# infergo-ml/gogp

Hardware: AMD Instinct MI355X
Metric: GP.Observe+Gradient evals/sec (fp64) at N=16384 D=8 (higher is better)
Workload: dtype f64

## Files before the change

### gogp_amd/_lib.py

```python
from __future__ import annotations

import ctypes
import os
import subprocess

from .kernel import CDesc

_HERE = os.path.dirname(os.path.abspath(__file__))
LIB_PATH = os.path.join(_HERE, "libgogp_hip.so")
HOOKS_PATH = os.path.join(_HERE, "libgogp_testhooks.so")

GOGP_OK, GOGP_EARG, GOGP_ENOTPD, GOGP_EHIP, GOGP_ESTATE, GOGP_ENOMEM, GOGP_ECOND = 0, 1, 2, 3, 4, 5, 6
GOGP_MAX_CANDIDATES = 16
GOGP_BATCH_MAX_N = 128
GOGP_COV_MAX_M = 4096

_dp = ctypes.POINTER(ctypes.c_double)
_i64 = ctypes.c_int64
_h = ctypes.c_void_p
_descp = ctypes.POINTER(CDesc)
GOGP_UNIQUE_ID_BYTES = 128


class CXfer(ctypes.Structure):
    _fields_ = [("peer", ctypes.c_int32), ("is_send", ctypes.c_int32), ("buf", ctypes.c_void_p),
                ("bytes", ctypes.c_int64)]


EXCHANGE_FN = ctypes.CFUNCTYPE(ctypes.c_int, ctypes.c_void_p, ctypes.POINTER(CXfer), ctypes.c_int32)
ALLREDUCE_FN = ctypes.CFUNCTYPE(ctypes.c_int, ctypes.c_void_p, ctypes.POINTER(ctypes.c_double),
                                ctypes.c_int64)
class CGemmOpts(ctypes.Structure):
    _fields_ = [(n, ctypes.c_int32) for n in ("ktri", "krag0", "new_row0", "kbeg0", "small_below", "prio", "rule",
                                              "tpb_shift", "rblk0", "cblk0", "pr", "Pr", "pc", "Pc", "beta0", "k")]
    _fields_ += [("bstride", ctypes.c_int64)]
    DEFAULTS = dict(ktri=0, krag0=-1, new_row0=-1, kbeg0=0, small_below=384, prio=0, rule=0, tpb_shift=0, rblk0=0,
                    cblk0=0, pr=0, Pr=1, pc=0, Pc=1, beta0=-1, k=1, bstride=0)


class CKParams(ctypes.Structure):
    _T, _D, _E = 4, 64, 32
    _fields_ = [("ndim", ctypes.c_int32), ("nterms", ctypes.c_int32), ("kind", ctypes.c_int32 * _T),
                ("ard", ctypes.c_int32 * _T), ("c", ctypes.c_double * _T), ("w", ctypes.c_double * _T),
                ("inv_len", (ctypes.c_double * _D) * _T), ("noise_var", ctypes.c_double), ("dnoise", ctypes.c_double),
                ("nevents", ctypes.c_int32), ("ev_axis", ctypes.c_int32), ("ev_from", ctypes.c_double * _E),
                ("ev_to", ctypes.c_double * _E), ("ev_disc", ctypes.c_double * _E)]


GOGP_TEST_NACC = 16 + 64


class CGemmPlan(ctypes.Structure):
    _fields_ = [("tile", ctypes.c_int32), ("waves", ctypes.c_int32), ("grid_x", ctypes.c_int64),
                ("grid_z", ctypes.c_int64), ("flops", ctypes.c_double), ("tag", ctypes.c_int64)]


SYMBOLS = [
    ("gogp_desc_check", ctypes.c_int, [_descp]),
    ("gogp_desc_ntheta_noise", ctypes.c_int, [_descp]),
    ("gogp_create", ctypes.c_int, [_descp, ctypes.c_int, ctypes.POINTER(_h)]),
    ("gogp_destroy", None, [_h]),
    ("gogp_last_error", ctypes.c_char_p, [_h]),
    ("gogp_notpd_index", _i64, [_h]),
    ("gogp_graph_info", ctypes.c_int, [_h, ctypes.POINTER(ctypes.c_int64), ctypes.POINTER(ctypes.c_int)]),
    ("gogp_events_check", ctypes.c_int, [_dp, ctypes.c_int, ctypes.c_int, ctypes.c_int]),
    ("gogp_set_events", ctypes.c_int, [_h, _dp, ctypes.c_int, ctypes.c_int]),
    ("gogp_set_data", ctypes.c_int, [_h, _dp, _dp, _i64]),
    ("gogp_set_data_device", ctypes.c_int, [_h, ctypes.c_void_p, ctypes.c_void_p, _i64]),
    ("gogp_absorb", ctypes.c_int, [_h, _dp, _dp]),
    ("gogp_observe", ctypes.c_int, [_h, _dp, _i64, _dp]),
    ("gogp_observe_full", ctypes.c_int, [_h, _dp, _i64, _dp]),
    ("gogp_lml", ctypes.c_int, [_h, _dp]),
    ("gogp_gradient", ctypes.c_int, [_h, _dp, _i64]),
    ("gogp_loo", ctypes.c_int, [_h, _dp, _dp, _dp, _dp]),
    ("gogp_loo_gradient", ctypes.c_int, [_h, _dp, _i64]),
    ("gogp_observe_gradient_batch", ctypes.c_int,
     [ctypes.POINTER(_h), ctypes.c_int, _dp, _i64, _dp, _dp, ctypes.POINTER(ctypes.c_int)]),
    ("gogp_observe_gradient_candidates", ctypes.c_int,
     [_h, ctypes.c_int, _dp, _i64, _dp, _dp, ctypes.POINTER(ctypes.c_int)]),
    ("gogp_batch_set_data", ctypes.c_int,
     [_h, _dp, _dp, _i64, ctypes.c_int32, ctypes.POINTER(_i64), ctypes.POINTER(_i64)]),
    ("gogp_batch_observe_gradient", ctypes.c_int,
     [_h, ctypes.c_int32, ctypes.POINTER(ctypes.c_int32), _dp, _i64, _dp, _dp, ctypes.POINTER(ctypes.c_int)]),
    ("gogp_batch_produce", ctypes.c_int,
     [_h, ctypes.c_int32, ctypes.POINTER(ctypes.c_int32), _dp, _i64, ctypes.POINTER(_i64), _dp, _dp, _dp, _dp,
      ctypes.POINTER(ctypes.c_int)]),
    ("gogp_batch_observe_full_gradient", ctypes.c_int,
     [_h, ctypes.c_int32, _dp, ctypes.POINTER(_i64), _dp, _dp, ctypes.POINTER(ctypes.c_int)]),
    ("gogp_batch_produce_full", ctypes.c_int,
     [_h, ctypes.c_int32, _dp, ctypes.POINTER(_i64), ctypes.POINTER(_i64), _dp, _dp, _dp, _dp,
      ctypes.POINTER(ctypes.c_int)]),
    ("gogp_produce", ctypes.c_int, [_h, _dp, _i64, _dp, _dp]),
    ("gogp_produce_gradient", ctypes.c_int, [_h, _dp, _i64, _dp, _dp, _dp, _dp]),
    ("gogp_produce_covariance", ctypes.c_int, [_h, _dp, _i64, _dp, _dp]),
    ("gogp_produce_samples", ctypes.c_int, [_h, _dp, _i64, _dp, _i64, ctypes.c_double, _dp, _dp]),
    ("gogp_n", _i64, [_h]),
    ("gogp_get_alpha", ctypes.c_int, [_h, _dp]),
    ("gogp_get_factor", ctypes.c_int, [_h, _dp]),
    ("gogp_get_factor_rows", ctypes.c_int, [_h, ctypes.POINTER(_i64), _i64, _dp]),
    ("gogp_get_factor_diag", ctypes.c_int, [_h, _dp]),
    ("gogp_set_factor", ctypes.c_int, [_h, _dp, _dp, _dp, _dp]),
    ("gogp_append", ctypes.c_int, [_h, _dp, _dp, ctypes.c_int64]),
    ("gogp_remove", ctypes.c_int, [_h, ctypes.POINTER(_i64), ctypes.c_int64]),
    ("gogp_dist_grid", ctypes.c_int, [ctypes.c_int, ctypes.POINTER(ctypes.c_int), ctypes.POINTER(ctypes.c_int)]),
    ("gogp_dist_unique_id", ctypes.c_int, [ctypes.c_void_p]),
    ("gogp_dist_init_rccl", ctypes.c_int,
     [_h, ctypes.c_int, ctypes.c_int, ctypes.c_int, ctypes.c_int, ctypes.c_char_p]),
    ("gogp_dist_init_callbacks", ctypes.c_int,
     [_h, ctypes.c_int, ctypes.c_int, ctypes.c_int, ctypes.c_int, ctypes.c_void_p, ctypes.c_void_p,
      ctypes.c_void_p]),
    ("gogp_dist_local_bytes", _i64, [_h]),
    ("gogp_dist_comm_ranks", ctypes.c_int, [_h, ctypes.POINTER(ctypes.c_int)]),
    ("gogp_dist_selftest", ctypes.c_int, [_h, ctypes.c_int, _i64]),
    ("gogp_profile_enable", ctypes.c_int, [_h, ctypes.c_int]),
    ("gogp_profile_read", ctypes.c_int, [_h, _dp, ctypes.POINTER(_i64), _dp, _dp]),
    ("gogp_profile_read_launches", ctypes.c_int,
     [_h, _i64, _dp, _dp, _dp, ctypes.POINTER(_i64), ctypes.POINTER(_i64)]),
    ("gogp_profile_read_aux", ctypes.c_int, [_h, ctypes.c_int, _dp, ctypes.POINTER(_i64)]),
    ("gogp_set_option", ctypes.c_int, [_h, ctypes.c_char_p, _i64]),
    ("gogp_version", ctypes.c_char_p, []),
# ... 107 lines not shown
```

### gogp_amd/csrc/api.hip

```cpp
#include <math.h>
#include <stdio.h>
#include <stdlib.h>
#include <string.h>

#include <algorithm>
#include <initializer_list>
#include <mutex>
#include <new>
#include <thread>
#include <type_traits>
#include <utility>

#include "handle.h"

using namespace gogp;

static thread_local std::string g_create_error;

extern "C" int gogp_desc_ntheta_noise(const gogp_desc *d) {
  return (d && (d->noise_kind == GOGP_NOISE_UNIFORM || d->noise_kind == GOGP_NOISE_CONSTANT_PARAM)) ? 1 : 0;
}

extern "C" int gogp_desc_check(const gogp_desc *d) {
  if (!d) return GOGP_EARG;
  if (d->ndim < 1 || d->ndim > GOGP_MAX_NDIM) return GOGP_EARG;
  if (d->nterms < 1 || d->nterms > GOGP_MAX_TERMS) return GOGP_EARG;
  if (d->ntheta_simil < 1 || d->ntheta_simil > GOGP_MAX_NDIM + 8) return GOGP_EARG;
  if (d->noise_kind != GOGP_NOISE_CONSTANT && d->noise_kind != GOGP_NOISE_UNIFORM &&
      d->noise_kind != GOGP_NOISE_CONSTANT_PARAM)
    return GOGP_EARG;
  int nard = 0;
  for (int t = 0; t < d->nterms; ++t) {
    const gogp_term &T = d->terms[t];
    if (T.kind < GOGP_K_NORMAL || T.kind > GOGP_K_PERIODIC) return GOGP_EARG;
    if (T.scale_idx >= d->ntheta_simil || T.scale_idx < -1) return GOGP_EARG;
    const int nlen = T.ard ? d->ndim : 1;
    if (T.len_idx < 0 || T.len_idx + nlen > d->ntheta_simil) return GOGP_EARG;
    if (T.kind == GOGP_K_PERIODIC) {
      if (T.period_idx < 0 || T.period_idx >= d->ntheta_simil) return GOGP_EARG;
      if (!(T.period_mult > 0)) return GOGP_EARG;
    }
    if (T.ard) ++nard;
  }
  if (nard > 1) return GOGP_EARG;
  return GOGP_OK;
}

extern "C" int gogp_events_check(const double *events, int nevents, int axis, int ndim) {
  if (nevents < 0 || nevents > GOGP_MAX_EVENTS) return GOGP_EARG;
  if (ndim < 1 || ndim > GOGP_MAX_NDIM || axis < 0 || axis >= ndim) return GOGP_EARG;
  if (nevents > 0 && !events) return GOGP_EARG;
  for (int i = 0; i < 3 * nevents; ++i)
    if (!isfinite(events[i])) return GOGP_EARG;
  return GOGP_OK;
}

extern "C" const char *gogp_version(void) {
#ifndef GOGP_BUILD_ID
#define GOGP_BUILD_ID "unknown"
#endif
  return "gogp_hip 0.3 gfx950 fp64-mfma(v_mfma_f64_16x16x4_f64) tile128 panel256 build " GOGP_BUILD_ID;
}

extern "C" const char *gogp_last_error(const gogp_handle *h) {
  if (!h) return g_create_error.c_str();
  return h->err.c_str();
}

extern "C" int64_t gogp_notpd_index(const gogp_handle *h) { return h ? h->notpd : -1; }
extern "C" int64_t gogp_n(const gogp_handle *h) { return h ? h->n : 0; }

static void free_n_buffers(gogp_handle *h) {
  nbufs_free(nbufs_of(h));
  nbufs_put(h, NBufs());
  (void)hipFree(h->bufY);
  h->bufY = nullptr;
  (void)hipFree(h->rw);
  (void)hipFree(h->rz);
  (void)hipFree(h->rd);
  (void)hipFree(h->rpart);
  h->small_ws.release();
  h->app_ws.release();
  h->rm_ws.release();
  h->loo_vec.release();
  h->loo_mat.release();
  (void)hipFree(h->TX);
  (void)hipFree(h->Tmt);
  h->TX = h->Tmt = nullptr;
  h->cap_tinv = 0;
  h->tinv_valid = h->tinv_pending = false;
  (void)hipFree(h->g32A);
  (void)hipFree(h->g32L);
  (void)hipFree(h->g32Y);
  (void)hipFree(h->g32D);
  h->g32A = h->g32L = h->g32Y = h->g32D = nullptr;
  h->g32_cap = 0;
  h->rw = h->rz = h->rd = h->rpart = nullptr;
  h->cap_npad = 0;
  h->cap_y = 0;
}

static void drop_cand_graph(gogp_handle *h) {
  if (h->cand_graph) (void)hipGraphExecDestroy(h->cand_graph);
  h->cand_graph = nullptr;
  h->cand_seen_key = CandGraphKey();
}
static hipError_t graph_stream(gogp_handle *h);

static void free_cand_buffers(gogp_handle *h) {
  drop_cand_graph(h);
  (void)hipFree(h->cand_arena);
  (void)hipHostFree(h->cand_hostP);
  (void)hipHostFree(h->cand_hscal);
  h->cand_arena = nullptr;
  h->cand_hostP = nullptr;
  h->cand_hscal = nullptr;
  h->cand_stride = 0;
  h->cand_cap_k = h->cand_host_k = 0;
  h->cand_cap_npad = 0;
}

static void free_m_buffers(gogp_handle *h) {
  (void)hipFree(h->dZ);
  (void)hipFree(h->KsT);
  (void)hipFree(h->Vt);
  (void)hipFree(h->pvec);
  h->pg_ws.release();
  h->pc_ws.release();
  h->dZ = h->KsT = h->Vt = h->pvec = nullptr;
  h->cap_m = h->cap_mp_npad = 0;
}

struct StreamSet {
  int device = -1;
  bool in_use = false;
  hipStream_t s = nullptr, s2 = nullptr, sp = nullptr, st = nullptr, sl = nullptr, sk = nullptr;
  hipStream_t sg = nullptr;
};
static std::mutex g_pool_mutex;
static std::vector<StreamSet *> g_stream_pool;

static hipError_t create_stream_set(StreamSet *ss, int device) {
  ss->device = device;
  hipError_t e = hipSuccess;
  e = hipStreamCreateWithFlags(&ss->s, hipStreamNonBlocking);
  if (e == hipSuccess) e = hipStreamCreateWithFlags(&ss->s2, hipStreamNonBlocking);
  if (e == hipSuccess) {
    int least = 0, greatest = 0;
    (void)hipDeviceGetStreamPriorityRange(&least, &greatest);
    const int normal = (least + greatest) / 2;
    e = hipStreamCreateWithPriority(&ss->sp, hipStreamNonBlocking, greatest);
    if (e == hipSuccess) e = hipStreamCreateWithPriority(&ss->st, hipStreamNonBlocking, normal);
    if (e == hipSuccess) e = hipStreamCreateWithPriority(&ss->sl, hipStreamNonBlocking, normal);
    if (e == hipSuccess) e = hipStreamCreateWithPriority(&ss->sk, hipStreamNonBlocking, least);
  }
  return e;
}

static hipError_t acquire_streams(gogp_handle *h, int device) {
  std::lock_guard<std::mutex> lock(g_pool_mutex);
  StreamSet *ss = nullptr;
  for (StreamSet *c : g_stream_pool)
    if (!c->in_use && c->device == device) {
      ss = c;
      break;
    }
  if (!ss) {
    ss = new StreamSet();
    const hipError_t e = create_stream_set(ss, device);
    if (e != hipSuccess) {
      for (hipStream_t q : {ss->s, ss->s2, ss->sp, ss->st, ss->sl, ss->sk})
        if (q) (void)hipStreamDestroy(q);
      delete ss;
      return e;
    }
    g_stream_pool.push_back(ss);
  }
  ss->in_use = true;
  h->stream_set = ss;
  h->s = ss->s;
  h->s2 = ss->s2;
  h->sp = ss->sp;
  h->st = ss->st;
  h->sl = ss->sl;
  h->sk = ss->sk;
  return hipSuccess;
}

static hipError_t graph_stream(gogp_handle *h) {
  StreamSet *ss = static_cast<StreamSet *>(h->stream_set);
  if (!ss->sg) {
    const hipError_t e = hipStreamCreateWithFlags(&ss->sg, hipStreamNonBlocking);
    if (e != hipSuccess) return e;
  }
  h->sg = ss->sg;
  return hipSuccess;
}

static void release_streams(gogp_handle *h) {
  std::lock_guard<std::mutex> lock(g_pool_mutex);
  if (h->stream_set) static_cast<StreamSet *>(h->stream_set)->in_use = false;
  h->stream_set = nullptr;
// ... 161 lines not shown
    for (int f = 0; f < 3; ++f) h->events[e][f] = events[3 * e + f];
  h->factored = h->have_alpha = h->have_kinv = h->observed = h->grad_valid = false;
  h->trtri_done = h->trtri_pending = h->alpha_pending = h->kinv_pending = false;
  h->tinv_valid = h->tinv_pending = false;
  return GOGP_OK;
}

static void fill_params_theta(const gogp_handle *h, const double *ts, const double *tn, DevParams &p) {
  const gogp_desc &d = h->desc;
  memset(&p, 0, sizeof p);
  p.ndim = d.ndim;
  p.nterms = d.nterms;
  p.ns = h->ns;
  p.nn = h->nn;
  for (int t = 0; t < d.nterms; ++t) {
    const gogp_term &T = d.terms[t];
    p.kind[t] = T.kind;
    p.ard[t] = T.ard;
    p.c[t] = T.scale_idx >= 0 ? ts[T.scale_idx] : 1.0;
    p.w[t] = 0.0;
    if (T.kind == GOGP_K_PERIODIC)
      p.w[t] = M_PI / (T.period_mult * ts[T.period_idx]);
    for (int j = 0; j < d.ndim; ++j)
      p.inv_len[t][j] = 1.0 / ts[T.len_idx + (T.ard ? j : 0)];
  }
  if (d.noise_kind == GOGP_NOISE_CONSTANT || d.noise_kind == GOGP_NOISE_CONSTANT_PARAM) {
    p.noise_var = d.noise_std * d.noise_std;
    p.dnoise = 0.0;
  } else {
    const double sd = tn[0];
    p.noise_var = d.noise_scale * sd * sd;
    p.dnoise = 2.0 * p.noise_var;
  }
  p.nevents = h->nevents;
  p.ev_axis = h->ev_axis;
  for (int e = 0; e < h->nevents; ++e) {
    p.ev_from[e] = h->events[e][0];
    p.ev_to[e] = h->events[e][1];
    p.ev_disc[e] = h->events[e][2];
  }
}

static void fill_params(const gogp_handle *h, DevParams &p) {
  fill_params_theta(h, h->theta_s.data(), h->theta_n.data(), p);
}

int gogp_upload_params(gogp_handle *h) {
  if (h->batch_mode) return GOGP_OK;
  fill_params(h, *h->hostP);
  HIPCHK(h, hipMemcpyAsync(h->devP, h->hostP, sizeof(DevParams), hipMemcpyHostToDevice, h->s));
  return GOGP_OK;
}

static hipError_t cand_memset(gogp_handle *h, void *dst, size_t bytes, hipStream_t s) {
  hipError_t e = hipSuccess;
  for (int c = 0; c < h->batch_k && e == hipSuccess; ++c)
    e = gogp::rec_memset_async((char *)dst + (size_t)c * h->cand_stride, 0, bytes, s);
  return e;
}
static hipError_t cand_copy_in(gogp_handle *h, void *dst, const void *src, size_t bytes, hipStream_t s) {
  hipError_t e = hipSuccess;
  for (int c = 0; c < h->batch_k && e == hipSuccess; ++c)
    e = gogp::rec_memcpy_async((char *)dst + (size_t)c * h->cand_stride, src, bytes, hipMemcpyDeviceToDevice, s);
  return e;
}
static hipError_t cand_d2h(gogp_handle *h, double *hdst, const void *dsrc, size_t bytes, hipStream_t s) {
  hipError_t e = hipSuccess;
  for (int c = 0; c < h->batch_k && e == hipSuccess; ++c)
    e = gogp::rec_memcpy_async(hdst + (size_t)c * BATCH_ROW, (const char *)dsrc + (size_t)c * h->cand_stride, bytes,
                               hipMemcpyDeviceToHost, s);
  return e;
}

static int ensure_y(gogp_handle *h) {
  if (h->bufY && h->cap_y >= h->npad) return GOGP_OK;
  (void)hipFree(h->bufY);
  h->bufY = nullptr;
  h->cap_y = 0;
  const int64_t cap = std::max(h->npad, h->cap_npad);
  HIPCHK(h, hipMalloc(&h->bufY, (size_t)cap * (size_t)cap * h->esz()));
  h->cap_y = cap;
  return GOGP_OK;
}

static int ensure_d64(gogp_handle *h) {
  if (h->D64 && h->cap_d64 >= h->npad) return GOGP_OK;
  (void)hipFree(h->D64);
  h->D64 = nullptr;
  h->cap_d64 = 0;
  const int64_t cap = std::max(h->npad, h->cap_npad);
  HIPCHK(h, hipMalloc(&h->D64, (size_t)cap * PANEL * sizeof(double)));
  h->cap_d64 = cap;
  return GOGP_OK;
}

struct FactorResult {
  int rc = GOGP_OK;
  double lml = 0.0, cond_lb = 1.0, yta = 0.0;
  int64_t notpd = -1;
  std::string msg;
};
static FactorResult judge_scalars(const gogp_handle *h, const double *hs, bool fp32, bool refine, int64_t n = -1) {
  FactorResult r;
  long long info = 0;
  memcpy(&info, hs + HS_INFO, sizeof info);
  char buf[160];
  if (info != 0) {
    r.rc = GOGP_ENOTPD;
    r.notpd = (int64_t)info - 1;
    snprintf(buf, sizeof buf, "Factorize: matrix is not positive definite (pivot %lld)", (long long)r.notpd);
    r.msg = buf;
    return r;
  }
  const double logdet = fp32 ? hs[5] : hs[0];
  const double ztz = refine ? hs[6] : hs[1];
  r.yta = ztz;
  r.lml = -0.5 * (double)(n < 0 ? h->n : n) * log(2 * M_PI) - 0.5 * logdet - 0.5 * ztz;
  const double dmin = hs[3], dmax = hs[4];
  r.cond_lb = (dmin > 0.0) ? (dmax / dmin) * (dmax / dmin) : INFINITY;
  if (!(r.cond_lb <= h->cond_limit)) {
    snprintf(buf, sizeof buf, "Condition: matrix singular or near-singular with condition number >= %.4e",
             r.cond_lb);
    r.msg = buf;
    r.rc = GOGP_ECOND;
  }
  return r;
}

static int finish_factorize(gogp_handle *h, bool fp32, bool refine, bool kinv) {
  h->alpha_pending = true;
  if (h->batch_mode) {
    h->factored = h->have_alpha = true;
    if (kinv) h->have_kinv = true;
    return GOGP_OK;
  }
  HIPCHK(h, hipStreamSynchronize(h->s));
  HIPCHK(h, hipGetLastError());
  const FactorResult fr = judge_scalars(h, h->hscal, fp32, refine);
  if (fr.rc == GOGP_ENOTPD) {
    h->alpha_pending = h->kinv_pending = false;
    h->tinv_valid = h->tinv_pending = false;
    h->trtri_done = h->trtri_pending = false;
    h->notpd = fr.notpd;
    h->err = fr.msg;
    return GOGP_ENOTPD;
  }
  h->lml = fr.lml;
  h->yta = fr.yta;
  h->factored = h->have_alpha = true;
  h->z_valid = true;
  if (kinv) h->have_kinv = true;
  h->cond_lb = fr.cond_lb;
  if (fr.rc == GOGP_ECOND) h->err = fr.msg;
  return fr.rc;
}

static void diag_block(gogp_handle *h, hipStream_t sp, const double *A, int64_t ld, double *L, int64_t ldl,
                       double *Dp, int64_t c0) {
  launch_diag256(sp, A, ld, L, ldl, Dp, c0, h->n, h->info);
}
static void diag_block(gogp_handle *h, hipStream_t sp, const float *A, int64_t ld, float *L, int64_t ldl,
                       float *Dp, int64_t c0) {
  double *A64 = h->dscr, *L64 = h->dscr + PANEL * PANEL, *D64 = h->dscr + 2 * PANEL * PANEL;
  if (h->d64_active)
    A64 = h->D64 + (size_t)(c0 / PANEL) * PANEL * PANEL;
  else
    launch_convert_block(sp, A, ld, A64, PANEL, PANEL, PANEL);
  launch_diag256(sp, A64, PANEL, L64, PANEL, D64, c0, h->n, h->info);
  launch_convert_block(sp, L64, PANEL, L, ldl, PANEL, PANEL);
  launch_convert_block(sp, D64, PANEL, Dp, PANEL, PANEL, PANEL);
  launch_logdet_block(sp, L64, PANEL, c0, h->n, PANEL, h->scalars + 5);
}
static void diag_inv_only(gogp_handle *h, hipStream_t s, const double *L, int64_t ld, double *Dp) {
  (void)h;
  launch_diag256_inv_only(s, L, ld, Dp);
}
static void diag_inv_only(gogp_handle *h, hipStream_t s, const float *L, int64_t ld, float *Dp) {
  double *L64 = h->dscr + PANEL * PANEL, *D64 = h->dscr + 2 * PANEL * PANEL;
  launch_convert_block(s, L, ld, L64, PANEL, PANEL, PANEL);
  launch_diag256_inv_only(s, L64, PANEL, D64);
  launch_convert_block(s, D64, PANEL, Dp, PANEL, PANEL, PANEL);
}

static inline int chain_prio_of(const gogp_handle *h) {
  return h->chain_prio < 0 ? (h->npad <= 6144 ? 1 : 0) : h->chain_prio;
}
static inline GemmGrid chain_grid(const gogp_handle *h) {
  GemmGrid g;
  g.prio = chain_prio_of(h);
  return g;
}

static inline int superpanel_width(const gogp_handle *h, int npanel, int P0) {
  const int head = h->superpanel_head < 0 ? (h->prec == 32 ? 4 : 3) : h->superpanel_head;
  const int sw = (head > 0 && npanel - P0 > h->head_remaining) ? head : h->superpanel;
  return (npanel - P0 < sw) ? npanel - P0 : sw;
}
struct SuperPanel {
  int P0, nsub, prevP0, next_nsub;
  int64_t C0() const { return (int64_t)P0 * PANEL; }
  int64_t CE() const { return C0() + (int64_t)nsub * PANEL; }
};
static std::vector<SuperPanel> superpanels(const gogp_handle *h) {
  const int npanel = (int)(h->npad / PANEL);
  std::vector<SuperPanel> v;
  for (int P0 = 0; P0 < npanel; P0 += v.back().nsub) {
    const int nsub = superpanel_width(h, npanel, P0);
    if (!v.empty()) v.back().next_nsub = nsub;
    v.push_back({P0, nsub, v.empty() ? -1 : v.back().P0, 0});
  }
  return v;
}
struct InnerGroup {
  int grp;
  int64_t k0, ce;
};
static inline InnerGroup inner_group(int q, int64_t c2, int64_t CE) {
  const int done = q + 1, grp = done & -done;
  return {grp, c2 - (int64_t)grp * PANEL, std::min(c2 + (int64_t)grp * PANEL, CE)};
}

constexpr int TMT_BLOCKS = 8;
static inline int tinv_panels(const gogp_handle *h) { return h->produce_panels; }
static inline int64_t tinv_signature(const gogp_handle *h) {
  return (int64_t)h->produce_panels + (h->npad << 8) + ((int64_t)h->prec << 56);
}
static int ensure_tinv(gogp_handle *h) {
  const int64_t tld = (int64_t)tinv_panels(h) * PANEL;
  const size_t need = (size_t)std::max(h->npad, h->cap_npad) * (size_t)tld;
  if (!h->TX || h->cap_tinv < need) {
    (void)hipFree(h->TX);
    (void)hipFree(h->Tmt);
    h->TX = h->Tmt = nullptr;
    h->cap_tinv = 0;
    HIPCHK(h, hipMalloc(&h->TX, need * h->esz()));
    HIPCHK(h, hipMalloc(&h->Tmt, (size_t)TMT_BLOCKS * PANEL * PANEL * h->esz()));
    h->cap_tinv = need;
  }
  h->tinv_ld = tld;
  return GOGP_OK;
}

template <class T>
static void assemble_tinv(gogp_handle *h, hipStream_t sp, int P0, int nsub) {
  const int64_t ld = h->npad, tld = h->tinv_ld, C0 = (int64_t)P0 * PANEL;
  T *X = reinterpret_cast<T *>(h->TX) + C0 * tld;
  T *MT = reinterpret_cast<T *>(h->Tmt);
  const T *L = reinterpret_cast<const T *>(h->bufL);
  const T *Dinv = reinterpret_cast<const T *>(h->Dinv) + (size_t)P0 * PANEL * PANEL;
  launch_tinv_init(sp, Dinv, X, (T *)nullptr, nsub, tld);
  for (int d = 1; d < nsub; ++d) {
    const int cnt = nsub - d;
    for (int b0 = 0; b0 < cnt; b0 += 6) {
      const int nb = std::min(6, cnt - b0);
      const T *A1[6], *B1[6], *A2[6], *B2[6];
      T *C1[6], *C2[6];
      int64_t lda1[6], ldb1[6], ldc1[6], lda2[6], ldb2[6], ldc2[6];
      int K1[6], K2[6];
      for (int b = 0; b < nb; ++b) {
        const int i = d + b0 + b, j = i - d;
        A1[b] = L + (C0 + (int64_t)i * PANEL) * ld + C0 + (int64_t)j * PANEL;
        lda1[b] = ld;
        B1[b] = X + (int64_t)j * PANEL * tld + (int64_t)j * PANEL;
        ldb1[b] = tld;
        C1[b] = MT + (size_t)(b0 + b) * PANEL * PANEL;
        ldc1[b] = PANEL;
        K1[b] = d * PANEL;
        A2[b] = Dinv + (size_t)i * PANEL * PANEL;
        lda2[b] = PANEL;
        B2[b] = C1[b];
        ldb2[b] = PANEL;
        C2[b] = X + (int64_t)i * PANEL * tld + (int64_t)j * PANEL;
        ldc2[b] = tld;
        K2[b] = PANEL;
      }
      launch_blockmm(sp, nb, A1, lda1, B1, ldb1, C1, ldc1, K1, 1.0);
      launch_blockmm(sp, nb, A2, lda2, B2, ldb2, C2, ldc2, K2, -1.0);
    }
  }
}

template <class T>
struct InvBufs {
  T *A, *Y;
  const T *L, *Dinv;
};
template <class T>
static void trtri_superstep(gogp_handle *h, const InvBufs<T> &B, const SuperPanel &P, hipStream_t st, hipStream_t s2) {
  const int64_t npad = h->npad, ld = npad;
  T *R = B.A, *Y = B.Y;
  const T *L = B.L;
  GemmProfile *pf = &h->prof;
  const int P0 = P.P0;
  const int64_t C0 = P.C0(), CE = P.CE();
  for (int q = 0; q < P.nsub; ++q) {
    const int p = P0 + q;
    const int64_t c0 = (int64_t)p * PANEL, c2 = c0 + PANEL;
    const T *Dp = B.Dinv + (size_t)p * PANEL * PANEL;
    launch_ydiag(st, Dp, Y + c0 * ld + c0, ld);
    if (c2 < CE)
      launch_zero_block(st, Y + c2 * ld + c0, ld, CE - c2, PANEL);
    if (c0 > 0) {
      GemmGrid gtri = chain_grid(h);
      gtri.ktri = h->ktri;
      launch_gemm_nt(st, GEMM_RECT, (int)(c0 / TILE), 2, PANEL, 1.0, R + c0, ld, Dp, PANEL, 0.0,
                      Y + c0, ld, pf, &gtri);
    }
    if (c2 < CE) {
      const InnerGroup g = inner_group(q, c2, CE);
      GemmGrid gch = chain_grid(h);
      if (h->krag) gch.krag0 = (int)(g.k0 / TILE);
      launch_gemm_nt(st, GEMM_RECT, (int)(c2 / TILE), (int)((g.ce - c2) / TILE), (int64_t)g.grp * PANEL,
                      -1.0, Y + g.k0, ld, L + c2 * ld + g.k0, ld, 1.0, R + c2, ld, pf, &gch);
    }
  }
  order(h, EV_BASE + 4 * P0 + 2, st, s2);
  const int nt = (int)((npad - CE) / TILE);
  if (nt > 0) {
    const int64_t Kw = CE - C0;
    const int mr = (int)(CE / TILE);
    const int ntn = nt < 2 * P.next_nsub ? nt : 2 * P.next_nsub;
    if (P0 > 0 && st != s2)
      (void)gogp::rec_stream_wait(st, ev(h, EV_BASE + 4 * P.prevP0 + 3));
    GemmGrid gch = chain_grid(h), gbulk;
    if (h->krag) gch.krag0 = gbulk.krag0 = (int)(C0 / TILE);
    launch_gemm_nt(st, GEMM_RECT, mr, ntn, Kw, -1.0, Y + C0, ld, L + CE * ld + C0, ld, 1.0,
                    R + CE, ld, pf, &gch);
    if (nt > ntn) {
      const int64_t C3 = CE + (int64_t)ntn * TILE;
      launch_gemm_nt(s2, GEMM_RECT, mr, nt - ntn, Kw, -1.0, Y + C0, ld, L + C3 * ld + C0, ld, 1.0,
                      R + C3, ld, pf, &gbulk);
    }
    (void)gogp::rec_event_record(ev(h, EV_BASE + 4 * P0 + 3), s2);
  }
}

static inline bool mixed_gradient(const gogp_handle *h) {
  return h->grad_prec == 32 && h->prec == 64 && !h->batch_mode && !h->dist;
}
static int ensure_g32(gogp_handle *h) {
  const int64_t cap = std::max(h->npad, h->cap_npad);
  if (h->g32A && h->g32_cap >= cap) return GOGP_OK;
  (void)hipFree(h->g32A);
  (void)hipFree(h->g32L);
  (void)hipFree(h->g32Y);
  (void)hipFree(h->g32D);
  h->g32A = h->g32L = h->g32Y = h->g32D = nullptr;
  h->g32_cap = 0;
  const size_t nn = (size_t)cap * (size_t)cap * sizeof(float);
  HIPCHK(h, hipMalloc(&h->g32A, nn));
  HIPCHK(h, hipMalloc(&h->g32L, nn));
  HIPCHK(h, hipMalloc(&h->g32Y, nn));
  HIPCHK(h, hipMalloc(&h->g32D, (size_t)(cap / PANEL) * PANEL * PANEL * sizeof(float)));
  h->g32_cap = cap;
  return GOGP_OK;
}
static void mixed_superstep(gogp_handle *h, const SuperPanel &P, hipStream_t st, hipStream_t s2) {
  const int64_t npad = h->npad, ld = npad, C0 = P.C0(), W = P.CE() - C0;
  launch_convert_block(st, h->bufL + C0 * ld + C0, ld, h->g32L + C0 * ld + C0, ld, (int)(npad - C0), (int)W);
  launch_convert_block(st, h->Dinv + (size_t)P.P0 * PANEL * PANEL, PANEL, h->g32D + (size_t)P.P0 * PANEL * PANEL, PANEL,
                       (int)W, PANEL);
  const InvBufs<float> B{h->g32A, h->g32Y, h->g32L, h->g32D};
  trtri_superstep<float>(h, B, P, st, s2);
}

template <class T>
static void kinv_accumulate(gogp_handle *h, const T *Y, T *A, int64_t C0, int64_t CE) {
  (void)gogp::rec_stream_wait(h->sk, ev(h, EV_BASE + 4 * (size_t)(C0 / PANEL) + 2));
  GemmGrid gk;
  gk.new_row0 = (int)(C0 / TILE);
  if (h->krag) gk.krag0 = (int)(C0 / TILE);
  launch_gemm_nt(h->sk, GEMM_LOWER, (int)(CE / TILE), (int)(CE / TILE), CE - C0, 1.0, Y + C0, h->npad, Y + C0, h->npad,
                 1.0, A, h->npad, &h->prof, &gk);
}

template <class T>
static void zero_inverse_rhs(gogp_handle *h, bool mixed, hipStream_t s) {
  if (mixed)
    launch_zero_upper_blocks(s, h->g32A, h->npad, h->npad);
  else
    launch_zero_upper_blocks(s, reinterpret_cast<T *>(h->bufA), h->npad, h->npad);
}
template <class T>
static void inverse_superstep(gogp_handle *h, bool mixed, const SuperPanel &P, hipStream_t st, hipStream_t s2,
                              bool fuse_kinv) {
  if (mixed) {
    mixed_superstep(h, P, st, s2);
    if (fuse_kinv) kinv_accumulate<float>(h, h->g32Y, h->g32A, P.C0(), P.CE());
  } else {
    const InvBufs<T> B{reinterpret_cast<T *>(h->bufA), reinterpret_cast<T *>(h->bufY), reinterpret_cast<const T *>(h->bufL),
                       reinterpret_cast<const T *>(h->Dinv)};
    trtri_superstep<T>(h, B, P, st, s2);
    if (fuse_kinv) kinv_accumulate<T>(h, B.Y, B.A, P.C0(), P.CE());
  }
}

static inline int chain_split_of(const gogp_handle *h, bool eager) {
  if (h->dist || h->prec != 64) return 0;
  if (h->chain_split >= 0) return h->chain_split;
  return (h->npad <= 8192 || !eager) ? 2 : 0;
}
static void fused_panel(gogp_handle *h, hipStream_t sp, double *A, double *L, int64_t ld, int64_t c0, int64_t npad,
                        GemmProfile *pf) {
  const int64_t c1 = c0 + TILE, c2 = c0 + PANEL;
  const int mt1 = (int)((npad - c1) / TILE);
  const GemmGrid gch = chain_grid(h);
  launch_panel128_slabs(sp, A + c0 * ld + c0, ld, L + c0 * ld + c0, ld, 0, npad - c1, c0, h->n, h->info, h->chain_slabs);
  launch_gemm_nt(sp, GEMM_RECT, mt1, 1, TILE, -1.0, L + c1 * ld + c0, ld, L + c1 * ld + c0, ld, 1.0, A + c1 * ld + c1, ld,
                 pf, &gch);
  launch_panel128_slabs(sp, A + c0 * ld + c0, ld, L + c0 * ld + c0, ld, 1, npad - c2, c0, h->n, h->info, h->chain_slabs);
}

static void begin_evaluation(gogp_handle *h, std::initializer_list<hipStream_t> streams) {
  auto wait = [&](int e) {
    for (hipStream_t q : streams) (void)gogp::rec_stream_wait(q, ev(h, e));
  };
  if (h->trtri_pending) wait(EV_TRTRI);
  if (h->kinv_pending) wait(EV_KINV);
  if (h->kinv_c1 > 0 && !h->have_kinv) wait(EV_KINV);
  h->trtri_pending = h->kinv_pending = false;
  h->factored = h->have_alpha = h->have_kinv = h->grad_valid = false;
  h->alpha_pending = h->trtri_done = h->ydone_valid = h->d64_active = false;
  h->notpd = -1;
  h->kinv_c1 = 0;
  if (!h->batch_mode) h->tinv_valid = false;
}
static hipError_t enqueue_result_scalars(gogp_handle *h, hipStream_t s) {
  const hipError_t e = cand_d2h(h, h->hscal, h->scalars, 7 * sizeof(double), s);
  return e != hipSuccess ? e : cand_d2h(h, h->hscal + HS_INFO, h->info, sizeof(long long), s);
}

template <class T>
static void substitute_fwd(gogp_handle *h, hipStream_t q, const T *L, const T *Dinv, double *w, double *dst) {
  const int npanel = (int)(h->npad / PANEL);
  for (int b = 0; b < npanel; ++b) launch_trsv_fwd_step(q, L, h->npad, Dinv, b, npanel, w, dst);
}
template <class T>
static hipError_t substitute_bwd(gogp_handle *h, hipStream_t q, const T *L, const T *Dinv, const double *src, double *w,
                                 double *dst) {
  const int npanel = (int)(h->npad / PANEL);
  const hipError_t e = hipMemcpyAsync(w, src, (size_t)h->npad * sizeof(double), hipMemcpyDeviceToDevice, q);
  for (int b = npanel - 1; b >= 0 && e == hipSuccess; --b) launch_trsv_bwd_step(q, L, h->npad, Dinv, b, npanel, w, dst);
  return e;
}

template <class T>
struct Sweep {
  static constexpr bool fp32 = sizeof(T) == 4;
  gogp_handle *h;
  bool eager;
  T *A = reinterpret_cast<T *>(h->bufA), *L = reinterpret_cast<T *>(h->bufL), *Dinv = reinterpret_cast<T *>(h->Dinv);
  int64_t npad = h->npad, ld = npad;
  int npanel = (int)(npad / PANEL);
  GemmProfile *pf = &h->prof;
  hipStream_t s = h->s, st = h->st, s2 = h->s2;
  hipStream_t sp = h->lookahead ? h->sp : h->s;
  hipStream_t sz = h->lookahead ? h->sl : sp;
  bool mixed = !fp32 && mixed_gradient(h);
  bool fuse_kinv = eager && (h->kinv_fused < 0 ? (npad <= 10240 || mixed) : h->kinv_fused != 0);
  int split = fp32 ? 0 : chain_split_of(h, eager);

  void d64_init(hipStream_t q, int first, int nblk) const {
    if constexpr (fp32)
      launch_widen_diag_blocks(q, A + (int64_t)first * PANEL * (ld + 1), ld, h->D64 + (size_t)first * PANEL * PANEL, nblk);
  }
  void d64_update(hipStream_t q, int64_t k0, int64_t K, int first, int nblk) const {
    if constexpr (fp32) {
      if (h->d64_active)
        launch_diag_syrk_f64(q, L + (int64_t)first * PANEL * ld + k0, ld, K, h->D64 + (size_t)first * PANEL * PANEL, nblk);
    }
  }

  int build_gram() const {
    if (sp != s) order(h, EV_ENTRY, s, sp);
    HIPCHK(h, cand_memset(h, h->info, sizeof(long long), sp));
    const int w0 = superpanel_width(h, npanel, 0);
    {
      AuxTimer tm(h, GOGP_PROF_GRAM, s);
      launch_gram_lower_split(sp, s, h->devP, h->D, h->dX, h->n, npad, A, ld, (int64_t)w0 * PANEL, h->ev());
    }
    h->d64_active = fp32 && h->diag_fp64 != 0;
    if (h->d64_active) {
      const int rc = ensure_d64(h);
      if (rc != GOGP_OK) return rc;
      d64_init(sp, 0, w0);
      if (npanel > w0) d64_init(s, w0, npanel - w0);
    }
    (void)gogp::rec_event_record(ev(h, EV_GRAM), s);
    if (eager) {
      (void)gogp::rec_stream_wait(s2, ev(h, EV_GRAM));
      (void)gogp::rec_stream_wait(st, ev(h, EV_GRAM));
      zero_inverse_rhs<T>(h, mixed, s2);
      order(h, EV_INIT, s2, st);
    }
    return GOGP_OK;
  }

  void chain_superpanel(const SuperPanel &P) const {
    const int64_t CE = P.CE();
    for (int q = 0; q < P.nsub; ++q) {
      const int p = P.P0 + q;
      const int64_t c0 = (int64_t)p * PANEL, c2 = c0 + PANEL;
      if constexpr (!fp32) {
        if (split) fused_panel(h, sp, A, L, ld, c0, npad, pf);
      }
      if (!split) {
        T *Dp = Dinv + (size_t)p * PANEL * PANEL;
        diag_block(h, sp, A + c0 * ld + c0, ld, L + c0 * ld + c0, ld, Dp, c0);
        const int mt2 = (int)((npad - c2) / TILE);
        if (mt2 > 0) {
          GemmGrid gtri = chain_grid(h);
          gtri.ktri = h->ktri;
          launch_gemm_nt(sp, GEMM_RECT, mt2, 2, PANEL, 1.0, A + c2 * ld + c0, ld, Dp, PANEL, 0.0,
                          L + c2 * ld + c0, ld, pf, &gtri);
        }
      }
      if (c2 < CE) {
        d64_update(sp, c0, PANEL, p + 1, (int)((CE - c2) / PANEL));
        const InnerGroup g = inner_group(q, c2, CE);
        const GemmGrid gch = chain_grid(h);
        launch_gemm_nt(sp, GEMM_TRAP, (int)((npad - c2) / TILE), (int)((g.ce - c2) / TILE),
                        (int64_t)g.grp * PANEL, -1.0, L + c2 * ld + g.k0, ld, L + c2 * ld + g.k0, ld, 1.0,
                        A + c2 * ld + c2, ld, pf, &gch);
      }
    }
  }

  void panels_final(const SuperPanel &P) const {
    order(h, EV_BASE + 4 * P.P0, sp, s);
    if (sz != sp) (void)gogp::rec_stream_wait(sz, ev(h, EV_BASE + 4 * P.P0));
    if constexpr (!fp32) {
      if (split) {
        launch_dinv256_blocks(sz, L + (int64_t)P.P0 * PANEL * (ld + 1), ld, Dinv + (size_t)P.P0 * PANEL * PANEL, P.nsub);
        if (eager) {
          (void)gogp::rec_event_record(ev(h, EV_BASE + 5 * (size_t)npanel + 32 + (size_t)P.P0), sz);
          (void)gogp::rec_stream_wait(st, ev(h, EV_BASE + 5 * (size_t)npanel + 32 + (size_t)P.P0));
        }
      }
    }
    for (int q = 0; q < P.nsub; ++q) launch_trsv_fwd_step(sz, L, ld, Dinv, P.P0 + q, npanel, h->w, h->z);
  }

  void trailing_update(const SuperPanel &P) const {
    const int64_t C0 = P.C0(), CE = P.CE();
    const int mtE = (int)((npad - CE) / TILE);
    if (mtE <= 0) return;
    const int64_t Kw = CE - C0;
    const int ntn = mtE < 2 * P.next_nsub ? mtE : 2 * P.next_nsub;
    (void)gogp::rec_stream_wait(sp, ev(h, P.P0 > 0 ? EV_BASE + 4 * P.prevP0 + 1 : EV_GRAM));
    const GemmGrid gch = chain_grid(h);
    launch_gemm_nt(sp, GEMM_TRAP, mtE, ntn, Kw, -1.0, L + CE * ld + C0, ld, L + CE * ld + C0, ld,
                    1.0, A + CE * ld + CE, ld, pf, &gch);
    d64_update(sp, C0, Kw, (int)(CE / PANEL), ntn / 2);
    if (mtE > ntn) {
      const int64_t C3 = CE + (int64_t)ntn * TILE;
      launch_gemm_nt(s, GEMM_LOWER, mtE - ntn, mtE - ntn, Kw, -1.0, L + C3 * ld + C0, ld,
                      L + C3 * ld + C0, ld, 1.0, A + C3 * ld + C3, ld, pf);
      d64_update(s, C0, Kw, (int)(C3 / PANEL), (mtE - ntn) / 2);
    }
    (void)gogp::rec_event_record(ev(h, EV_BASE + 4 * P.P0 + 1), s);
  }

  void inverse_behind(const SuperPanel &P) const {
    const int64_t CE = P.CE();
    (void)gogp::rec_stream_wait(st, ev(h, EV_BASE + 4 * P.P0));
    inverse_superstep<T>(h, mixed, P, st, s2, fuse_kinv);
    if (!fp32 && !fuse_kinv && !mixed && !h->batch_mode && h->kinv_split > 0 && h->kinv_c1 == 0 && CE < npad &&
        CE * 100 >= npad * (int64_t)h->kinv_split) {
      (void)gogp::rec_stream_wait(h->sk, ev(h, EV_BASE + 4 * P.P0 + 2));
      const T *Y0 = reinterpret_cast<const T *>(h->bufY);
      launch_gemm_nt(h->sk, GEMM_LAUUM, (int)(CE / TILE), (int)(CE / TILE), CE, 1.0, Y0, ld, Y0, ld, 0.0, A, ld, pf);
      (void)gogp::rec_event_record(ev(h, EV_KINV), h->sk);
      h->kinv_c1 = CE;
    }
  }

  int finish_alpha() const {
    if (fp32) {
      if (sz != sp) (void)gogp::rec_stream_wait(sp, ev(h, EV_FWD));
      HIPCHK(h, substitute_bwd(h, sp, L, Dinv, h->z, h->w, h->alpha));
      for (int it = 0; it < h->refine_steps; ++it) {
        launch_residual(sp, h->devP, h->D, h->dX, h->n, npad, h->alpha, h->dy, h->rpart, REFINE_SLABS, h->rw,
                        h->radial1, h->ev());
        substitute_fwd(h, sp, L, Dinv, h->rw, h->rz);
        HIPCHK(h, substitute_bwd(h, sp, L, Dinv, h->rz, h->rw, h->rd));
        launch_axpy(sp, h->alpha, h->rd, npad);
      }
      launch_dot(sp, h->dy, h->alpha, h->n, h->scalars + 6);
      order(h, EV_ALPHA, sp, s);
    }
    HIPCHK(h, enqueue_result_scalars(h, s));
    if (fp32) {
      if (eager) (void)gogp::rec_event_record(ev(h, EV_TRTRI), st);
    } else if (eager && !mixed) {
      (void)gogp::rec_stream_wait(st, ev(h, EV_FWD));
      launch_alpha_from_y(st, reinterpret_cast<const T *>(h->bufY), ld, h->z, npad, h->alpha);
      (void)gogp::rec_event_record(ev(h, EV_ALPHA), st);
      (void)gogp::rec_event_record(ev(h, EV_TRTRI), st);
    } else {
      if (sz != sp) (void)gogp::rec_stream_wait(sp, ev(h, EV_FWD));
      HIPCHK(h, substitute_bwd(h, sp, L, Dinv, h->z, h->w, h->alpha));
      (void)gogp::rec_event_record(ev(h, EV_ALPHA), sp);
    }
    return GOGP_OK;
  }
};

template <class T>
static int factorize_t(gogp_handle *h, bool eager) {
  const Sweep<T> c{h, eager && h->lookahead != 0};
  begin_evaluation(h, {c.s, c.sp});
  int rc = gogp_upload_params(h);
  if (rc == GOGP_OK && (c.mixed || c.eager)) rc = c.mixed ? ensure_g32(h) : ensure_y(h);
  if (rc == GOGP_OK) rc = c.build_gram();
  if (rc != GOGP_OK) return rc;
  if (c.fp32) HIPCHK(h, hipMemsetAsync(h->scalars + 5, 0, sizeof(double), c.sp));
  HIPCHK(h, cand_copy_in(h, h->w, h->dy, (size_t)c.npad * sizeof(double), c.sp));
  if (c.sz != c.sp) order(h, EV_W, c.sp, c.sz);
  for (const SuperPanel &P : superpanels(h)) {
    c.chain_superpanel(P);
    c.panels_final(P);
    c.trailing_update(P);
    if (c.eager) c.inverse_behind(P);
  }
  if (c.fuse_kinv) {
    (void)gogp::rec_event_record(ev(h, EV_KINV), h->sk);
    h->kinv_pending = true;
  }
  if (c.eager) {
    (void)gogp::rec_event_record(ev(h, EV_TRTRI), c.st);
    (void)gogp::rec_event_record(ev(h, EV_YDONE), c.st);
    h->ydone_valid = h->trtri_done = h->trtri_pending = true;
  }
  order(h, EV_FWD, c.sz, c.s);
  launch_lml_scalars(c.s, c.L, c.ld, h->z, nullptr, nullptr, h->n, h->scalars);
  rc = c.finish_alpha();
  if (rc != GOGP_OK) return rc;
  const int rcf = finish_factorize(h, c.fp32, c.fp32, false);
  if (rcf == GOGP_ENOTPD)
    for (hipStream_t q : {c.sp, c.st, c.s2, h->sl, h->sk}) (void)hipStreamSynchronize(q);
  return rcf;
}

static inline bool tiny_ok(const gogp_handle *h) {
  return h->tiny && !h->dist && h->prec == 64 && h->npad == PANEL && h->n <= TILE && !mixed_gradient(h);
}
static int tiny_factorize(gogp_handle *h, bool eager) {
  hipStream_t s = h->s;
  begin_evaluation(h, {s});
  int rc = gogp_upload_params(h);
  if (rc != GOGP_OK) return rc;
  if (h->lookahead && !h->batch_mode) {
    order(h, EV_ENTRY, h->sp, s);
    order(h, EV_W, h->sl, s);
  }
  HIPCHK(h, cand_memset(h, h->info, sizeof(long long), s));
  launch_tiny_eval(s, h->devP, h->dX, h->dy, h->n, h->bufA, h->bufL, h->Dinv, h->z, h->alpha, h->info, eager, h->ev());
  launch_lml_scalars(s, h->bufL, h->npad, h->z, nullptr, nullptr, h->n, h->scalars);
  (void)gogp::rec_event_record(ev(h, EV_ALPHA), s);
  HIPCHK(h, enqueue_result_scalars(h, s));
  return finish_factorize(h, false, false, eager);
}

static int factorize(gogp_handle *h, bool eager) {
  if (tiny_ok(h)) return tiny_factorize(h, eager && h->lookahead);
  return h->prec == 32 ? factorize_t<float>(h, eager) : factorize_t<double>(h, eager);
}

static int ensure_alpha(gogp_handle *h) {
  if (!h->factored || !h->have_alpha) return fail(h, GOGP_ESTATE, "no factorisation");
  if (h->alpha_pending) {
    HIPCHK(h, gogp::rec_stream_wait(h->s, ev(h, EV_ALPHA)));
    h->alpha_pending = false;
  }
  return GOGP_OK;
}

static const char *theta_refusal(const gogp_handle *h, const double *ts, const double *tn) {
  for (int i = 0; i < h->ns; ++i)
    if (!(ts[i] > 0.0) || !std::isfinite(ts[i])) return "similarity parameters must be positive and finite";
  for (int i = 0; i < h->nn; ++i)
    if (!std::isfinite(tn[i])) return "noise parameter must be finite";
  return nullptr;
}

static int set_theta_natural(gogp_handle *h, const double *ts, const double *tn) {
  if (const char *why = theta_refusal(h, ts, tn)) return fail(h, GOGP_EARG, why);
  for (int i = 0; i < h->ns; ++i) h->theta_s[i] = ts[i];
  for (int i = 0; i < h->nn; ++i) h->theta_n[i] = tn[i];
  h->have_theta = true;
  return GOGP_OK;
}

extern "C" int gogp_absorb(gogp_handle *h, const double *theta_simil,
                           const double *theta_noise) {
  if (!h || !theta_simil || (h->nn > 0 && !theta_noise)) return fail(h, GOGP_EARG, "absorb: NULL");
// ... 12 lines not shown
  rc = h->dist ? gogp_dist_factorize(h, false) : factorize(h, false);
  if (rc != GOGP_OK && rc != GOGP_ECOND) return rc;
  const int rcond = rc;
  rc = ensure_alpha(h);
  if (rc != GOGP_OK) return rc;
  HIPCHK(h, hipStreamSynchronize(h->s));
  return rcond;
}

static int observe_theta(gogp_handle *h, const double *x, double *lml) {
  std::vector<double> th(h->P > 0 ? h->P : 1);
  for (int i = 0; i < h->P; ++i) th[i] = exp(x[i]);
  int rc = set_theta_natural(h, th.data(), th.data() + h->ns);
  if (rc != GOGP_OK) return rc;
  h->grad_valid = false;
  if (h->n == 0) {
    h->lml = 0.0;
    h->factored = false;
    h->observed = true;
    if (lml) *lml = 0.0;
    return GOGP_OK;
  }
  rc = h->dist ? gogp_dist_factorize(h, true)
               : factorize(h, h->eager != 0);
  if (rc != GOGP_OK && rc != GOGP_ECOND) return rc;
  h->observed = true;
  if (lml) *lml = h->lml;
  return rc;
}

extern "C" int gogp_observe(gogp_handle *h, const double *x, int64_t len, double *lml) {
  if (!h || !x) return fail(h, GOGP_EARG, "observe: NULL");
  if (len != h->P) return fail(h, GOGP_EARG, "len(x)");
  if (!h->have_data) return fail(h, GOGP_ESTATE, "observe: no data (gogp_set_data)");
  HIPCHK(h, hipSetDevice(h->device));
  h->with_obs = false;
  return observe_theta(h, x, lml);
}

extern "C" int gogp_observe_full(gogp_handle *h, const double *x, int64_t len, double *lml) {
  if (!h || !x) return fail(h, GOGP_EARG, "observe: NULL");
  if (len < h->P) return fail(h, GOGP_EARG, "len(x)");
  const int64_t rest = len - h->P;
  if (rest == 0) return gogp_observe(h, x, len, lml);
  const int64_t n = rest / (h->D + 1);
  if (n * (h->D + 1) != rest) return fail(h, GOGP_EARG, "len(x)");
  int rc = gogp_set_data(h, x + h->P, x + h->P + n * h->D, n);
  if (rc != GOGP_OK) return rc;
  h->with_obs = true;
  return observe_theta(h, x, lml);
}

extern "C" int gogp_lml(gogp_handle *h, double *lml) {
  if (!h || !lml) return GOGP_EARG;
  if (h->n == 0) {
    *lml = 0.0;
    return GOGP_OK;
  }
  if (!h->factored) return fail(h, GOGP_ESTATE, "LML: nothing absorbed");
  *lml = h->lml;
  return GOGP_OK;
}

template <class T>
static int compute_kinv_t(gogp_handle *h) {
  if (h->have_kinv) return GOGP_OK;
  const int64_t npad = h->npad, ld = npad;
  hipStream_t s = h->s;
  GemmProfile *pf = &h->prof;
  if (h->kinv_pending) {
    (void)gogp::rec_stream_wait(s, ev(h, EV_KINV));
    if (h->trtri_pending) (void)gogp::rec_stream_wait(s, ev(h, EV_TRTRI));
    h->kinv_pending = h->trtri_pending = false;
    h->have_kinv = true;
    return GOGP_OK;
  }
  const bool mixed = std::is_same<T, double>::value && mixed_gradient(h);
  if (!h->trtri_done) {
    hipStream_t sp = h->lookahead ? h->sp : h->s;
    const int rcy = mixed ? ensure_g32(h) : ensure_y(h);
    if (rcy != GOGP_OK) return rcy;
    zero_inverse_rhs<T>(h, mixed, s);
    order(h, EV_INIT, s, sp);
    for (const SuperPanel &P : superpanels(h)) inverse_superstep<T>(h, mixed, P, sp, s, false);
    order(h, EV_TRTRI, sp, s);
    h->trtri_done = true;
  } else if (h->trtri_pending) {
    (void)gogp::rec_stream_wait(s, ev(h, h->ydone_valid ? EV_YDONE : EV_TRTRI));
  }
  if (mixed) {
    launch_gemm_nt(s, GEMM_LAUUM, h->nblk, h->nblk, npad, 1.0, h->g32Y, ld, h->g32Y, ld, 0.0, h->g32A, ld, pf);
  } else {
    GemmGrid gk;
    if (h->kinv_c1 > 0) {
      (void)gogp::rec_stream_wait(s, ev(h, EV_KINV));
      gk.kbeg0 = (int)h->kinv_c1;
    }
    launch_gemm_nt(s, GEMM_LAUUM, h->nblk, h->nblk, npad, 1.0, reinterpret_cast<const T *>(h->bufY), ld,
                   reinterpret_cast<const T *>(h->bufY), ld, 0.0, reinterpret_cast<T *>(h->bufA), ld, pf, &gk);
  }
  if (h->trtri_pending && h->ydone_valid) (void)gogp::rec_stream_wait(s, ev(h, EV_TRTRI));
  h->trtri_pending = false;
  h->have_kinv = true;
  return GOGP_OK;
}
static int compute_kinv(gogp_handle *h) {
  return h->prec == 32 ? compute_kinv_t<float>(h) : compute_kinv_t<double>(h);
}

static int64_t grad_len(const gogp_handle *h) {
  return h->with_obs ? h->P + h->n * (h->D + 1) : h->P;
}

static void assemble_gradient(const gogp_handle *h, const double *a, double dnoise, double *out) {
  const gogp_desc &d = h->desc;
  for (int t = 0; t < d.nterms; ++t) {
    const gogp_term &T = d.terms[t];
    if (T.scale_idx >= 0) out[T.scale_idx] += 0.5 * a[3 * t + 0];
    if (T.ard) {
      for (int j = 0; j < d.ndim; ++j) out[T.len_idx + j] += 0.5 * a[ACC_ARD0 + j];
    } else {
      out[T.len_idx] += 0.5 * a[3 * t + 1];
    }
    if (T.kind == GOGP_K_PERIODIC) out[T.period_idx] += 0.5 * a[3 * t + 2];
  }
  if (h->nn > 0) out[h->ns] = 0.5 * a[ACC_TRACE] * dnoise;
}

static void fp32_gradient_identities(const gogp_handle *h, double *a, double trace_w, double yta, double noise_var) {
  const gogp_desc &d = h->desc;
  a[ACC_TRACE] = trace_w;
  if (d.nterms == 1 && d.terms[0].scale_idx >= 0) a[0] = (yta - (double)h->n) - noise_var * trace_w;
}

static int enqueue_grad_sums(gogp_handle *h, bool trace) {
  hipStream_t s = h->s;
  auto reduce = [&](auto *kinv) {
    AuxTimer tm(h, GOGP_PROF_GRAD, s);
    launch_grad_reduce(s, h->devP, h->D, h->ard_dims, h->dX, h->alpha, kinv, h->npad, h->n, h->npad, h->gpart, h->gout,
                       h->radial1, h->ard_mfma_min, h->ev());
  };
  if (h->prec == 32)
    reduce(reinterpret_cast<const float *>(h->bufA));
  else if (mixed_gradient(h))
    reduce((const float *)h->g32A);
  else
    reduce((const double *)h->bufA);
  HIPCHK(h, cand_d2h(h, h->hscal + HS_GRAD, h->gout, NACC * sizeof(double), s));
  h->hscal[HS_TRACE] = NAN;
  if (trace) {
    launch_trace_from_y(s, h->prec == 32 ? reinterpret_cast<const float *>(h->bufY) : (const float *)h->g32Y, h->npad, h->n,
                        h->npad, h->alpha, h->prec == 32 ? h->rw : h->w, h->scalars + 7);
    HIPCHK(h, hipMemcpyAsync(h->hscal + HS_TRACE, h->scalars + 7, sizeof(double), hipMemcpyDeviceToHost, s));
  }
  return GOGP_OK;
}

extern "C" int gogp_gradient(gogp_handle *h, double *grad, int64_t len) {
  if (!h || !grad) return fail(h, GOGP_EARG, "gradient: NULL");
  if (!h->observed) return fail(h, GOGP_ESTATE, "Gradient before Observe");
  if (len != grad_len(h)) return fail(h, GOGP_EARG, "gradient: wrong length");
  for (int64_t i = 0; i < len; ++i) grad[i] = 0.0;
  if (h->n == 0) return GOGP_OK;
  HIPCHK(h, hipSetDevice(h->device));
  if (h->dist && h->with_obs)
    return fail(h, GOGP_EARG, "sharded evaluation: the full Observe form is not supported");
  if (h->prec == 32 && h->with_obs)
// ... 107 lines not shown
  if (rc != GOGP_OK) return rc;
  for (int64_t i = 0; i < len; ++i) grad[i] = 0.0;
  if (empty) return GOGP_OK;
  hipStream_t s = h->s;
  const int64_t npad = h->npad, ld = npad;
  const size_t mat = (size_t)npad * (size_t)npad;
  rc = h->loo_mat.reserve(h, 2 * mat * sizeof(double));
  if (rc != GOGP_OK) return rc;
  double *B = h->loo_mat.as<double>(), *G = B + mat;
  launch_loo_scale_symv(s, h->bufA, ld, h->n, npad, lv.sc, lv.v, B, ld, G, lv.u);
  launch_gemm_nt(s, GEMM_LOWER, h->nblk, h->nblk, npad, 1.0, (const double *)B, ld, (const double *)B, ld, 0.0, G, ld,
                 &h->prof);
  launch_loo_rank2(s, G, ld, h->n, npad, lv.u, h->alpha);
  HIPCHK(h, hipMemsetAsync(lv.zero, 0, (size_t)npad * sizeof(double), s));
  {
    AuxTimer tm(h, GOGP_PROF_GRAD, s);
    launch_grad_reduce(s, h->devP, h->D, h->ard_dims, h->dX, lv.zero, (const double *)G, ld, h->n, npad, h->gpart, h->gout,
                       h->radial1, h->ard_mfma_min, h->ev());
  }
  double acc[NACC];
  HIPCHK(h, hipMemcpyAsync(acc, h->gout, sizeof acc, hipMemcpyDeviceToHost, s));
  HIPCHK(h, hipStreamSynchronize(s));
  HIPCHK(h, hipGetLastError());
  assemble_gradient(h, acc, h->hostP->dnoise, grad);
  return GOGP_OK;
}

static int fill_params_log(const gogp_handle *h, const double *x, DevParams &p) {
  std::vector<double> th((size_t)std::max(h->P, 1));
  for (int i = 0; i < h->P; ++i) th[(size_t)i] = exp(x[i]);
  int rc = GOGP_OK;
  if (theta_refusal(h, th.data(), th.data() + h->ns)) {
    rc = GOGP_EARG;
    std::fill(th.begin(), th.end(), 1.0);
  }
  fill_params_theta(h, th.data(), th.data() + h->ns, p);
  return rc;
}

static int judge_row(const gogp_handle *h, double *row, bool fp32, int64_t n, const DevParams &p, int st,
                     const char *refused, double *lml, double *g, int64_t len, std::string &first_msg) {
  *lml = NAN;
  if (g) std::fill(g, g + len, 0.0);
  if (st != GOGP_OK) {
    if (first_msg.empty()) first_msg = refused;
    return st;
  }
  const FactorResult fr = judge_scalars(h, row, fp32, fp32, n);
  if (fr.rc != GOGP_OK && first_msg.empty()) first_msg = fr.msg;
  if (fr.rc != GOGP_ENOTPD) {
    *lml = fr.lml;
    if (fp32 && std::isfinite(row[HS_TRACE]))
      fp32_gradient_identities(h, row + HS_GRAD, row[HS_TRACE], fr.yta, p.noise_var);
    if (g) assemble_gradient(h, row + HS_GRAD, p.dnoise, g);
  }
  return fr.rc;
}

extern "C" int gogp_observe_gradient_batch(gogp_handle **hs, int k, const double *xs, int64_t len,
                                           double *lmls, double *grads, int *status) {
  if (!hs || k <= 0 || !xs || !lmls || !grads) return GOGP_EARG;
  std::vector<int> st((size_t)k, GOGP_OK);
  auto body = [&](int i) {
    int rc = gogp_observe(hs[i], xs + (size_t)i * len, len, lmls + i);
    if (rc == GOGP_OK) rc = gogp_gradient(hs[i], grads + (size_t)i * len, len);
    st[(size_t)i] = rc;
  };
  std::vector<std::thread> th;
  for (int i = 1; i < k; ++i) th.emplace_back(body, i);
  body(0);
  for (auto &t : th) t.join();
  int first = GOGP_OK;
  for (int i = 0; i < k; ++i) {
    if (status) status[i] = st[(size_t)i];
    if (first == GOGP_OK && st[(size_t)i] != GOGP_OK) first = st[(size_t)i];
  }
  return first;
}

static size_t align_up(size_t v, size_t a) { return (v + a - 1) / a * a; }
constexpr int64_t GRAPH_MAX_NPAD = 1024;
constexpr int64_t GRAPH_EXPLICIT_MAX_NPAD = 8192;

static EvalBufs cand_layout(char *base, int64_t npad, size_t esz, size_t *bytes = nullptr) {
  EvalBufs b;
  size_t o = 0;
  auto take = [&](auto *&p, size_t n) {
    p = reinterpret_cast<std::remove_reference_t<decltype(p)>>(reinterpret_cast<uintptr_t>(base) + o);
    o += align_up(n, 256);
  };
  const size_t nn = (size_t)npad * (size_t)npad * esz;
  take(b.devP, sizeof(DevParams));
  take(b.info, sizeof(long long));
  take(b.scalars, 8 * sizeof(double));
  take(b.gout, NACC * sizeof(double));
  take(b.z, (size_t)npad * sizeof(double));
  take(b.w, (size_t)npad * sizeof(double));
  take(b.alpha, (size_t)npad * sizeof(double));
  take(b.gpart, (size_t)grad_reduce_blocks(npad) * NACC * sizeof(double));
  take(b.Dinv, (size_t)(npad / PANEL) * PANEL * PANEL * esz);
  take(b.bufA, nn);
  take(b.bufL, nn);
  take(b.bufY, nn);
  if (bytes) *bytes = align_up(o, 4096);
  return b;
}

static int ensure_candidates(gogp_handle *h, int k) {
  if (k > h->cand_host_k) {
    drop_cand_graph(h);
    (void)hipHostFree(h->cand_hostP);
    (void)hipHostFree(h->cand_hscal);
    h->cand_hostP = nullptr;
    h->cand_hscal = nullptr;
    h->cand_host_k = 0;
    HIPCHK(h, hipHostMalloc((void **)&h->cand_hostP, (size_t)k * sizeof(DevParams), hipHostMallocDefault));
    HIPCHK(h, hipHostMalloc((void **)&h->cand_hscal, (size_t)k * BATCH_ROW * sizeof(double), hipHostMallocDefault));
    h->cand_host_k = k;
  }
  if (k > h->cand_cap_k || h->npad > h->cand_cap_npad) {
    drop_cand_graph(h);
    (void)hipFree(h->cand_arena);
    h->cand_arena = nullptr;
    h->cand_cap_k = 0;
    h->cand_cap_npad = 0;
    const int64_t cap = std::max(h->npad, h->cand_cap_npad);
    size_t stride = 0;
    (void)cand_layout(nullptr, cap, h->esz(), &stride);
    HIPCHK(h, hipMalloc((void **)&h->cand_arena, stride * (size_t)k));
    h->cand_stride = stride;
    h->cand_cap_k = k;
    h->cand_cap_npad = cap;
  }
  return GOGP_OK;
}

static CandGraphKey cand_graph_key(const gogp_handle *h, int k) {
  return {k, h->n, h->cand_cap_npad, h->cand_stride, h->cand_arena, h->dX, h->dy, h->cand_hostP, h->cand_hscal};
}

extern "C" int gogp_observe_gradient_candidates(gogp_handle *h, int k, const double *xs, int64_t len,
                                                double *lmls, double *grads, int *status) {
  if (!h || k <= 0 || !xs || !lmls || !grads) return fail(h, GOGP_EARG, "candidates: bad arguments");
  if (k > GOGP_MAX_CANDIDATES) return fail(h, GOGP_EARG, "candidates: k > GOGP_MAX_CANDIDATES");
  if (len != h->P) return fail(h, GOGP_EARG, "len(x)");
  if (!h->have_data) return fail(h, GOGP_ESTATE, "candidates: no data (gogp_set_data)");
  if (h->dist) {
    HIPCHK(h, hipSetDevice(h->device));
    for (int c = 0; c < k; ++c) {
      lmls[c] = NAN;
      if (status) status[c] = GOGP_ESTATE;
      for (int64_t i = 0; i < len; ++i) grads[(size_t)c * len + i] = 0.0;
    }
    int first_d = GOGP_OK;
    for (int c = 0; c < k; ++c) {
      double *g = grads + (size_t)c * len;
      h->with_obs = false;
      int r = observe_theta(h, xs + (size_t)c * len, &lmls[c]);
      if (r == GOGP_OK || r == GOGP_ECOND) {
        const int rg = gogp_gradient(h, g, len);
        if (rg != GOGP_OK) r = rg;
      }
      if (r == GOGP_ENOTPD || r == GOGP_EARG) {
        lmls[c] = NAN;
        for (int64_t i = 0; i < len; ++i) g[i] = 0.0;
      } else if (r != GOGP_OK && r != GOGP_ECOND) {
        return r;
      }
      if (status) status[c] = r;
      if (first_d == GOGP_OK && r != GOGP_OK) first_d = r;
    }
    return first_d;
  }
  if (h->prec == 32 && k > 1) {
    int first32 = GOGP_OK;
    for (int c = 0; c < k; ++c) {
      const int r = gogp_observe_gradient_candidates(h, 1, xs + (size_t)c * len, len, lmls + c, grads + (size_t)c * len,
                                                     status ? status + c : nullptr);
      if (r != GOGP_OK && r != GOGP_ENOTPD && r != GOGP_ECOND && r != GOGP_EARG) return r;
      if (first32 == GOGP_OK && r != GOGP_OK) first32 = r;
    }
    return first32;
  }
  if (!h->lookahead || !h->eager)
    return fail(h, GOGP_EARG, "candidates: needs the fused sweep (options lookahead and eager on)");
  if (h->n == 0) {
    for (int c = 0; c < k; ++c) {
      lmls[c] = 0.0;
      if (status) status[c] = GOGP_OK;
      for (int64_t i = 0; i < len; ++i) grads[(size_t)c * len + i] = 0.0;
    }
    return GOGP_OK;
  }
  HIPCHK(h, hipSetDevice(h->device));
  for (hipStream_t q : work_streams(h)) HIPCHK(h, hipStreamSynchronize(q));
  if (h->kinv_pending) h->have_kinv = true;
  h->trtri_pending = h->alpha_pending = h->kinv_pending = h->tinv_pending = false;
  int rc = ensure_candidates(h, k);
  if (rc != GOGP_OK) return rc;

  const EvalBufs saved_bufs = *h;
  const EvalState saved_state = *h;
  double *const saved_hscal = h->hscal;
  const int64_t saved_cap_y = h->cap_y;
  static_cast<EvalBufs &>(*h) = cand_layout(h->cand_arena, h->cand_cap_npad, h->esz());
  h->hscal = h->cand_hscal;
  h->cap_y = h->cand_cap_npad;
  h->with_obs = false;
  h->batch_k = k;
  h->batch_mode = true;
  gogp::tl_batch.k = k;
  gogp::tl_batch.stride = (long)h->cand_stride;
  std::vector<int> st((size_t)k, GOGP_OK);

  for (int c = 0; c < k; ++c) st[(size_t)c] = fill_params_log(h, xs + (size_t)c * len, h->cand_hostP[c]);
  auto enqueue = [&]() -> int {
    for (int c = 0; c < k; ++c)
      HIPCHK(h, gogp::rec_memcpy_async((char *)h->devP + (size_t)c * h->cand_stride, h->cand_hostP + c,
                                       sizeof(DevParams), hipMemcpyHostToDevice, h->s));
    const bool f32 = h->prec == 32;
    int r = tiny_ok(h) ? tiny_factorize(h, true) : (f32 ? factorize_t<float>(h, true) : factorize_t<double>(h, true));
    if (r != GOGP_OK) return r;
    r = f32 ? compute_kinv_t<float>(h) : compute_kinv_t<double>(h);
    if (r != GOGP_OK) return r;
    r = ensure_alpha(h);
    if (r != GOGP_OK) return r;
    r = enqueue_grad_sums(h, f32 && h->trace_fp64);
    if (r != GOGP_OK) return r;
    size_t slot = EV_BASE + 4 * (size_t)(h->npad / PANEL);
    for (hipStream_t q : {h->sp, h->s2, h->st, h->sl, h->sk}) order(h, slot++, q, h->s);
    return GOGP_OK;
  };
  auto run = [&]() -> int {
    int r = GOGP_OK;
    const bool dag = h->use_graph >= 2;
    const bool graph = h->use_graph && h->prec == 64 && !h->prof.on && !h->graph_failed &&
                       h->npad <= (dag ? GRAPH_EXPLICIT_MAX_NPAD : GRAPH_MAX_NPAD);
    const CandGraphKey key = cand_graph_key(h, k);
    const bool hit = graph && h->cand_graph && h->cand_graph_key == key;
    const bool seen = graph && h->cand_seen_key == key;
    h->cand_seen_key = key;
    if (hit || seen) {
      if (!hit) {
        drop_cand_graph(h);
        HIPCHK(h, graph_stream(h));
        hipGraph_t gr = nullptr;
        hipError_t eg = hipSuccess;
        gogp::GraphRec rec;
        if (dag) {
          rec.chain = h->use_graph == 3;
          HIPCHK(h, hipGraphCreate(&rec.graph, 0));
          gogp::tl_rec = &rec;
          r = enqueue();
          gogp::tl_rec = nullptr;
          gr = rec.graph;
          eg = rec.err;
        } else {
          hipStream_t keep[6] = {h->s, h->sp, h->s2, h->st, h->sl, h->sk};
          h->s = h->sp = h->s2 = h->st = h->sl = h->sk = h->sg;
          eg = hipStreamBeginCapture(h->sg, hipStreamCaptureModeRelaxed);
          if (eg == hipSuccess) {
            r = enqueue();
            eg = hipStreamEndCapture(h->sg, &gr);
          }
          h->s = keep[0];
          h->sp = keep[1];
          h->s2 = keep[2];
          h->st = keep[3];
          h->sl = keep[4];
          h->sk = keep[5];
        }
        if (r == GOGP_OK && eg == hipSuccess) eg = hipGraphInstantiate(&h->cand_graph, gr, nullptr, nullptr, 0);
        if (gr) (void)hipGraphDestroy(gr);
        if (r != GOGP_OK) return r;
        if (eg != hipSuccess && dag) {
          (void)hipGetLastError();
          h->cand_graph = nullptr;
          h->graph_failed = true;
          h->graph_note = std::string("hipGraph not usable (") + hipGetErrorString(eg) + "): stream path";
          r = enqueue();
          if (r != GOGP_OK) return r;
          for (hipStream_t q : work_streams(h)) HIPCHK(h, hipStreamSynchronize(q));
          HIPCHK(h, hipGetLastError());
          return GOGP_OK;
        }
        HIPCHK(h, eg);
        if (dag) h->graph_nodes = rec.nodes;
        h->cand_graph_key = key;
      }
      HIPCHK(h, hipGraphLaunch(h->cand_graph, h->sg));
      HIPCHK(h, hipStreamSynchronize(h->sg));
    } else {
      r = enqueue();
      if (r != GOGP_OK) return r;
    }
    for (hipStream_t q : work_streams(h)) HIPCHK(h, hipStreamSynchronize(q));
    HIPCHK(h, hipGetLastError());
    return GOGP_OK;
  };
  rc = run();
  if (rc != GOGP_OK)
    for (hipStream_t q : work_streams(h)) (void)hipStreamSynchronize(q);

  std::string first_msg;
  int first = rc;
  if (rc == GOGP_OK) {
    for (int c = 0; c < k; ++c) {
      st[(size_t)c] = judge_row(h, h->hscal + (size_t)c * BATCH_ROW, h->prec == 32, h->n, h->cand_hostP[c], st[(size_t)c],
                                "candidates: parameters must be positive and finite", &lmls[c], grads + (size_t)c * len,
                                len, first_msg);
      if (first == GOGP_OK && st[(size_t)c] != GOGP_OK) first = st[(size_t)c];
    }
  }
  if (status)
    for (int c = 0; c < k; ++c) status[c] = (rc == GOGP_OK) ? st[(size_t)c] : rc;

  gogp::tl_batch.k = 1;
  gogp::tl_batch.stride = 0;
  h->batch_k = 1;
  h->batch_mode = false;
  static_cast<EvalBufs &>(*h) = saved_bufs;
  static_cast<EvalState &>(*h) = saved_state;
  h->hscal = saved_hscal;
  h->cap_y = saved_cap_y;
  h->trtri_pending = h->alpha_pending = h->kinv_pending = false;
  if (first != GOGP_OK && rc == GOGP_OK) h->err = first_msg;
  return first;
}

extern "C" int gogp_batch_set_data(gogp_handle *h, const double *X, const double *y, int64_t rows, int32_t nmembers,
                                   const int64_t *offset, const int64_t *n) {
  if (!h) return GOGP_EARG;
  if (h->dist) return fail(h, GOGP_EARG, "batch: not supported on a sharded handle");
  if (rows < 0 || nmembers < 0 || (rows > 0 && (!X || !y)) || (nmembers > 0 && (!offset || !n)))
    return fail(h, GOGP_EARG, "batch_set_data: bad arguments");
  for (int32_t b = 0; b < nmembers; ++b)
    if (n[b] < 0 || n[b] > GOGP_BATCH_MAX_N || offset[b] < 0 || offset[b] > rows - n[b])
      return fail(h, GOGP_EARG, "batch_set_data: every member needs 0 <= n <= GOGP_BATCH_MAX_N rows inside the data");
  HIPCHK(h, hipSetDevice(h->device));
  HIPCHK(h, hipStreamSynchronize(h->s));
  if (rows > h->bt_cap_rows || !h->bt_X) {
    (void)hipFree(h->bt_X);
    (void)hipFree(h->bt_y);
    h->bt_X = h->bt_y = nullptr;
    h->bt_cap_rows = 0;
    h->bt_have = false;
    const int64_t cap = std::max<int64_t>(rows, 1);
    HIPCHK(h, hipMalloc(&h->bt_X, ((size_t)cap * h->D + GOGP_MAX_NDIM) * sizeof(double)));
    HIPCHK(h, hipMalloc(&h->bt_y, (size_t)cap * sizeof(double)));
    h->bt_cap_rows = cap;
  }
  if (rows > 0) {
    HIPCHK(h, hipMemcpy(h->bt_X, X, (size_t)rows * h->D * sizeof(double), hipMemcpyHostToDevice));
    HIPCHK(h, hipMemcpy(h->bt_y, y, (size_t)rows * sizeof(double), hipMemcpyHostToDevice));
  }
  h->bt_rows = rows;
  h->bt_off.assign(offset, offset + nmembers);
  h->bt_n.assign(n, n + nmembers);
  h->bt_have = true;
  return GOGP_OK;
}

static int bt_reserve(gogp_handle *h, char **dev, char **host, size_t *cap, size_t bytes) {
  if (bytes <= *cap) return GOGP_OK;
  (void)hipFree(*dev);
  if (*host) (void)hipHostFree(*host);
  *dev = *host = nullptr;
  *cap = 0;
  HIPCHK(h, hipMalloc((void **)dev, bytes));
  HIPCHK(h, hipHostMalloc((void **)host, bytes, hipHostMallocDefault));
  *cap = bytes;
  return GOGP_OK;
}

static int batch_eval(gogp_handle *h, int32_t k, const int32_t *members, const double *x, int64_t len, const int64_t *xoff,
                      const int64_t *zoff, const double *Z, double *lmls, double *grads, double *mu, double *sigma,
                      int *status) {
  const bool produce = zoff != nullptr, full = xoff != nullptr;
  if (!h) return GOGP_EARG;
  if (h->dist) return fail(h, GOGP_EARG, "batch: not supported on a sharded handle");
  if (k < 0 || (k > 0 && ((!full && !members) || !x || !lmls || (!produce && !grads))))
    return fail(h, GOGP_EARG, "batch: bad arguments");
  int64_t nx = 0;
  if (full) {
    if (xoff[0] < 0) return fail(h, GOGP_EARG, "batch: xoff must be non-negative and non-decreasing");
    for (int32_t i = 0; i < k; ++i)
      if (xoff[i + 1] < xoff[i]) return fail(h, GOGP_EARG, "batch: xoff must be non-negative and non-decreasing");
    nx = xoff[k] - xoff[0];
  } else {
    if (len != h->P) return fail(h, GOGP_EARG, "len(x)");
    if (!h->bt_have) return fail(h, GOGP_ESTATE, "batch: no batch data (gogp_batch_set_data)");
    const int64_t nmem = (int64_t)h->bt_n.size();
    for (int32_t i = 0; i < k; ++i)
      if (members[i] < 0 || members[i] >= nmem) return fail(h, GOGP_EARG, "batch: member index out of range");
  }
  int64_t mz = 0;
  if (produce) {
    if (zoff[0] < 0) return fail(h, GOGP_EARG, "batch_produce: zoff must be non-negative and non-decreasing");
    for (int32_t i = 0; i < k; ++i)
      if (zoff[i + 1] < zoff[i]) return fail(h, GOGP_EARG, "batch_produce: zoff must be non-negative and non-decreasing");
    mz = zoff[k];
    if (mz > 0 && (!Z || !mu || !sigma)) return fail(h, GOGP_EARG, "batch_produce: bad arguments");
  }
  if (k == 0) return GOGP_OK;
  HIPCHK(h, hipSetDevice(h->device));
  const int64_t P = h->P, D = h->D;
  std::vector<int> st((size_t)k, GOGP_OK);
// ... 1041 lines not shown
  h->prof.used = 0;
  h->prof.flops = 0;
  h->prof.launches = 0;
  h->prof.lflops.clear();
  h->prof.ltag.clear();
  return GOGP_OK;
}

extern "C" int gogp_set_option(gogp_handle *h, const char *name, int64_t value) {
  if (!h || !name) return GOGP_EARG;
  drop_cand_graph(h);
  if (strcmp(name, "produce_tinv") == 0) {
    h->produce_tinv = value != 0;
    return GOGP_OK;
  }
  if (strcmp(name, "produce_panels") == 0) {
    if (value < 1 || value > 8) return fail(h, GOGP_EARG, "produce_panels must be 1..8");
    h->produce_panels = (int)value;
    return GOGP_OK;
  }
  if (strcmp(name, "produce_small_below") == 0) {
    if (value < 0) return fail(h, GOGP_EARG, "produce_small_below must be >= 0");
    h->produce_small_below = (int)value;
    return GOGP_OK;
  }
  if (strcmp(name, "produce_small_max") == 0) {
    if (value < 0 || value > 64) return fail(h, GOGP_EARG, "produce_small_max must be 0..64");
    h->produce_small_max = (int)value;
    return GOGP_OK;
  }
  if (strcmp(name, "produce_groups") == 0) {
    if (value < 1 || value > PRODUCE_GROUPS) return fail(h, GOGP_EARG, "produce_groups must be 1..4");
    h->produce_groups = (int)value;
    return GOGP_OK;
  }
  if (strcmp(name, "gradient_precision") == 0) {
    if (value != 32 && value != 64) return fail(h, GOGP_EARG, "gradient_precision must be 32 or 64");
    if (value == 32 && (h->desc.nterms != 1 || h->desc.terms[0].scale_idx < 0))
      return fail(h, GOGP_EARG, "gradient_precision = 32 is offered for one-term kernels with an output scale only");
    HIPCHK(h, hipSetDevice(h->device));
    for (hipStream_t q : work_streams(h)) HIPCHK(h, hipStreamSynchronize(q));
    h->grad_prec = (int)value;
    h->have_kinv = h->grad_valid = false;
    h->trtri_done = h->trtri_pending = h->kinv_pending = false;
    return GOGP_OK;
  }
  if (strcmp(name, "trace_fp64") == 0) {
    h->trace_fp64 = value != 0;
    return GOGP_OK;
  }
  if (strcmp(name, "krag") == 0) {
    h->krag = value != 0;
    return GOGP_OK;
  }
  if (strcmp(name, "lookahead") == 0) {
    h->lookahead = value != 0;
    return GOGP_OK;
  }
  if (strcmp(name, "eager") == 0) {
    h->eager = value != 0;
    return GOGP_OK;
  }
  if (strcmp(name, "precision") == 0) {
    if (value != 32 && value != 64) return fail(h, GOGP_EARG, "precision must be 32 or 64");
    if (h->dist && (int)value != h->prec)
      return fail(h, GOGP_EARG, "precision: set it before gogp_dist_init_* (the shard's buffers are typed)");
    if ((int)value != h->prec) {
      HIPCHK(h, hipSetDevice(h->device));
      for (hipStream_t q : work_streams(h)) HIPCHK(h, hipStreamSynchronize(q));
      free_n_buffers(h);
      free_m_buffers(h);
      free_cand_buffers(h);
      h->prec = (int)value;
      h->have_data = h->factored = h->have_alpha = h->have_kinv = h->observed = h->grad_valid = false;
      h->trtri_done = h->trtri_pending = h->alpha_pending = h->kinv_pending = false;
    }
    return GOGP_OK;
  }
  if (strcmp(name, "kinv_split") == 0) {
    if (value < 0 || value > 95) return fail(h, GOGP_EARG, "kinv_split must be 0..95");
    h->kinv_split = (int)value;
    return GOGP_OK;
  }
  if (strcmp(name, "kinv_fused") == 0) {
    h->kinv_fused = value < 0 ? -1 : (value != 0);
    return GOGP_OK;
  }
  if (strcmp(name, "superpanel_head") == 0) {
    if (value < -1 || value > 8) return fail(h, GOGP_EARG, "superpanel_head must be -1..8");
    h->superpanel_head = (int)value;
    return GOGP_OK;
  }
  if (strcmp(name, "head_remaining") == 0) {
    if (value < 0) return fail(h, GOGP_EARG, "head_remaining must be >= 0");
    h->head_remaining = (int)value;
    return GOGP_OK;
  }
  if (strcmp(name, "ard_mfma_min_dims") == 0) {
    if (value < 1 || value > 65) return fail(h, GOGP_EARG, "ard_mfma_min_dims must be 1..65");
    h->ard_mfma_min = (int)value;
    return GOGP_OK;
  }
  if (strcmp(name, "chain_prio") == 0) {
    if (value < -1 || value > 2) return fail(h, GOGP_EARG, "chain_prio must be -1..2");
    h->chain_prio = (int)value;
    return GOGP_OK;
  }
  if (strcmp(name, "tiny") == 0) {
    if (value < 0 || value > 1) return fail(h, GOGP_EARG, "tiny must be 0 or 1");
    h->tiny = (int)value;
    return GOGP_OK;
  }
  if (strcmp(name, "chain_slabs") == 0) {
    if (value < 0 || value > 8) return fail(h, GOGP_EARG, "chain_slabs must be 0..8");
    h->chain_slabs = (int)value;
    return GOGP_OK;
  }
  if (strcmp(name, "chain_split") == 0) {
    if (value < -1 || value > 2 || value == 1) return fail(h, GOGP_EARG, "chain_split must be -1, 0 or 2");
    h->chain_split = (int)value;
    return GOGP_OK;
  }
  if (strcmp(name, "ktri") == 0) {
    h->ktri = value != 0;
    return GOGP_OK;
  }
  if (strcmp(name, "graph") == 0) {
    if (value < 0 || value > 3) return fail(h, GOGP_EARG, "graph must be 0..3");
    h->use_graph = (int)value;
    h->graph_failed = false;
    drop_cand_graph(h);
    return GOGP_OK;
  }
  if (strcmp(name, "diag_fp64") == 0) {
    if (value < 0 || value > 1) return fail(h, GOGP_EARG, "diag_fp64 must be 0 or 1");
    h->diag_fp64 = (int)value;
    return GOGP_OK;
  }
  if (strcmp(name, "refine_steps") == 0) {
    if (value < 0 || value > 8) return fail(h, GOGP_EARG, "refine_steps must be 0..8");
    h->refine_steps = (int)value;
    return GOGP_OK;
  }
  if (strcmp(name, "cond_limit_log10") == 0) {
    if (value < 1 || value > 300) return fail(h, GOGP_EARG, "cond_limit_log10 must be 1..300");
    h->cond_limit = pow(10.0, (double)value);
    return GOGP_OK;
  }
  if (strcmp(name, "superpanel") == 0) {
    if (value < 1 || value > 8) return fail(h, GOGP_EARG, "superpanel must be 1..8");
    h->superpanel = (int)value;
    return GOGP_OK;
  }
  return fail(h, GOGP_EARG, "unknown option");
}
```

### gogp_amd/csrc/common.h

```cpp
#pragma once
#include <hip/hip_runtime.h>
#include <stdint.h>

#include <string>
#include <vector>

#include "../../include/gogp_hip.h"
#include "graphrec.h"

namespace gogp {

constexpr int TILE = 128;
constexpr int PANEL = 256;
constexpr int GEMM_BK = 16;

struct DevParams {
  int ndim, nterms, ns, nn;
  int kind[GOGP_MAX_TERMS];
  int ard[GOGP_MAX_TERMS];
  double c[GOGP_MAX_TERMS];
  double w[GOGP_MAX_TERMS];
  double inv_len[GOGP_MAX_TERMS][GOGP_MAX_NDIM];
  double noise_var;
  double dnoise;
  int nevents, ev_axis;
  double ev_from[GOGP_MAX_EVENTS], ev_to[GOGP_MAX_EVENTS], ev_disc[GOGP_MAX_EVENTS];
};

constexpr int ACC_TRACE = 3 * GOGP_MAX_TERMS;
constexpr int ACC_ARD0 = 16;
constexpr int NACC = ACC_ARD0 + GOGP_MAX_NDIM;

struct Batch {
  int k = 1;
  long stride = 0;
};
inline thread_local Batch tl_batch;
template <class P>
__device__ __forceinline__ P *cand(P *p, long bstride) {
  return (P *)((const char *)p + (long)blockIdx.z * bstride);
}

struct GemmProfile {
  bool on = false;
  std::vector<hipEvent_t> pool;
  size_t used = 0;
  double flops = 0;
  int64_t launches = 0;
  std::vector<double> lflops;
  std::vector<int64_t> ltag;
};

struct GemmGrid {
  int rule = 0, tpb_shift = 0, rblk0 = 0, cblk0 = 0, pr = 0, Pr = 1, pc = 0, Pc = 1, beta0 = -1;
  int new_row0 = -1;
  int ktri = 0;
  int prio = 0;
  int krag0 = -1;
  int small_below = 384;
  int kbeg0 = 0;
};

struct BlockMap {
  int nb_shift = 9, pr = 0, Pr = 1, pc = 0, Pc = 1;
  __host__ __device__ long grow(long lrow) const {
    const long nbm = (1L << nb_shift) - 1;
    return ((((lrow >> nb_shift) * Pr + pr)) << nb_shift) + (lrow & nbm);
  }
  __host__ __device__ long gcol(long lcol) const {
    const long nbm = (1L << nb_shift) - 1;
    return ((((lcol >> nb_shift) * Pc + pc)) << nb_shift) + (lcol & nbm);
  }
};

#ifdef GOGP_WGSTAMP
struct StampRec {
  long long base, nwg, tag, stream;
};
constexpr int STAMP_SLOTS = 8;
extern unsigned long long *g_stamp_buf;
extern long long g_stamp_cap, g_stamp_used, g_stamp_nrec;
extern StampRec g_stamp_rec[1 << 16];
unsigned long long *stamp_reserve(long long nwg, long long tag, hipStream_t s);
#endif

enum GemmMode { GEMM_RECT = 0, GEMM_LOWER = 1, GEMM_LAUUM = 2,
                GEMM_TRAP = 3 };

void launch_dgemm_nt(hipStream_t s, GemmMode mode, int mt, int nt, int64_t K,
                     double alpha, const double *A, int64_t lda, const double *B,
                     int64_t ldb, double beta, double *C, int64_t ldc,
                     GemmProfile *prof, const GemmGrid *grid = nullptr);

void launch_gemm_nt(hipStream_t s, GemmMode mode, int mt, int nt, int64_t K, double alpha, const double *A,
                    int64_t lda, const double *B, int64_t ldb, double beta, double *C, int64_t ldc,
                    GemmProfile *prof, const GemmGrid *grid = nullptr);
void launch_gemm_nt(hipStream_t s, GemmMode mode, int mt, int nt, int64_t K, double alpha, const float *A,
                    int64_t lda, const float *B, int64_t ldb, double beta, float *C, int64_t ldc,
                    GemmProfile *prof, const GemmGrid *grid = nullptr);
void launch_gram_lower_split(hipStream_t s_first, hipStream_t s_rest, const DevParams *p, int ndim,
                             const double *X, int64_t n, int64_t npad, float *K, int64_t ld,
                             int64_t wcols, bool ev = false);
void launch_cross(hipStream_t s, const DevParams *p, int ndim, const double *X, int64_t n,
                  int64_t npad, const double *Z, int64_t m, int64_t mpad, float *KsT, int64_t ld, bool ev = false);
void launch_trsv_fwd_step(hipStream_t s, const float *L, int64_t ld, const float *Dinv, int b, int nblk,
                          double *y, double *z);
void launch_trsv_bwd_step(hipStream_t s, const float *L, int64_t ld, const float *Dinv, int b, int nblk,
                          double *zwork, double *alpha);
void launch_lml_scalars(hipStream_t s, const float *L, int64_t ld, const double *z, const double *y,
                        const double *alpha, int64_t n, double *scalars);
void launch_alpha_from_y(hipStream_t s, const float *Y, int64_t ld, const double *z, int64_t npad,
                         double *alpha);
void launch_rownorm_dot(hipStream_t s, const float *V, int64_t ld, const double *vec, int64_t ncols,
                        int64_t m, double *dot, double *sq);
void launch_zero_upper_blocks(hipStream_t s, float *R, int64_t ld, int64_t npad);
void launch_zero_block(hipStream_t s, float *B, int64_t ld, int64_t rows, int64_t cols);
void launch_ydiag(hipStream_t s, const float *Dinv, float *Ydiag, int64_t ld);
void launch_extract_lower(hipStream_t s, const float *L, int64_t ld, int64_t n, double *out);
void launch_pack_lower(hipStream_t s, const double *in, int64_t n, int64_t npad, float *L, int64_t ld);
void launch_convert_block(hipStream_t s, const float *src, int64_t lds_, double *dst, int64_t ldd, int rows,
                          int cols);
void launch_convert_block(hipStream_t s, const double *src, int64_t lds_, float *dst, int64_t ldd, int rows,
                          int cols);
void launch_grad_reduce(hipStream_t s, const DevParams *p, int ndim, int ard_dims, const double *X,
                        const double *alpha, const float *Kinv, int64_t ld, int64_t n, int64_t npad,
                        double *partials, double *out, bool radial1 = false, int mfma_min_dims = 1, bool ev = false,
                        int max_blocks = 0);

void launch_gram_lower(hipStream_t s, const DevParams *p, int ndim, const double *X,
                       int64_t n, int64_t npad, double *K, int64_t ld, bool ev = false);
void launch_gram_local(hipStream_t s, const DevParams *p, int ndim, const double *X, int64_t n,
                       int64_t mrows, int64_t ncols, BlockMap map, double *K, int64_t ld, bool ev = false);
void launch_gram_local(hipStream_t s, const DevParams *p, int ndim, const double *X, int64_t n,
                       int64_t mrows, int64_t ncols, BlockMap map, float *K, int64_t ld, bool ev = false);
void launch_gram_lower_split(hipStream_t s_first, hipStream_t s_rest, const DevParams *p, int ndim,
                             const double *X, int64_t n, int64_t npad, double *K, int64_t ld,
                             int64_t wcols, bool ev = false);
void launch_cross(hipStream_t s, const DevParams *p, int ndim, const double *X, int64_t n,
                  int64_t npad, const double *Z, int64_t m, int64_t mpad, double *KsT,
                  int64_t ld, bool ev = false);
void launch_residual(hipStream_t s, const DevParams *p, int ndim, const double *X, int64_t n, int64_t npad,
                     const double *v, const double *y, double *part, int nslab, double *r, bool radial1 = false,
                     bool ev = false);
void launch_kmatvec_share(hipStream_t s, const DevParams *p, int ndim, const double *X, int64_t n, int64_t npad,
                          const double *v, int part_idx, int nparts, double *part, int nslab, double *out,
                          bool radial1 = false, bool ev = false);
void launch_prior(hipStream_t s, const DevParams *p, const double *Z, int64_t m,
                  double *prior);

void launch_trsv_fwd_step(hipStream_t s, const double *L, int64_t ld, const double *Dinv,
                          int b, int nblk, double *y, double *z);
void launch_trsv_bwd_step(hipStream_t s, const double *L, int64_t ld, const double *Dinv,
                          int b, int nblk, double *zwork, double *alpha);

void launch_lml_scalars(hipStream_t s, const double *L, int64_t ld, const double *z,
                        const double *y, const double *alpha, int64_t n, double *scalars);
void launch_diag256(hipStream_t s, const double *A, int64_t ld, double *Lout, int64_t ldl,
                    double *Dinv, int64_t row0, int64_t nvalid, long long *info);
void launch_diag256_ld512(hipStream_t s, const double *A, int64_t ld, double *Lout, int64_t ldl,
                          double *Dinv, int64_t row0, int64_t nvalid, long long *info);
void launch_diag256_inv_only(hipStream_t s, const double *L, int64_t ld, double *Dinv);
void launch_diag_syrk_f64(hipStream_t s, const float *Lrows, int64_t ld, int64_t K, double *D64, int nblocks);
void launch_widen_diag_blocks(hipStream_t s, const float *A, int64_t ld, double *D64, int nblocks);
void launch_diag_syrk_f64_tiles(hipStream_t s, const float *Lrows, int64_t ld, int64_t K, double *D64, int nblocks,
                                int64_t row_stride, int bs);
void launch_panel128(hipStream_t s, const double *A, int64_t ld, double *Lout, int64_t ldl, int half, int64_t rows_below,
                     int64_t row0, int64_t nvalid, long long *info);
void launch_panel128_slabs(hipStream_t s, const double *A, int64_t ld, double *Lout, int64_t ldl, int half,
                           int64_t rows_below, int64_t row0, int64_t nvalid, long long *info, int slabs);
void launch_tiny_eval(hipStream_t s, const DevParams *P, const double *X, const double *y, int64_t n, double *A, double *L,
                      double *Dinv, double *z, double *alpha, long long *info, bool want_kinv, bool ev = false);
struct BatchItem {
  DevParams P;
  long off, n;
  long zoff, m;
  long roff;
};
constexpr int BATCH_ROW = NACC + 16;
void launch_batch_eval(hipStream_t s, const BatchItem *items, int k, const double *X, const double *y, const double *Z,
                       double *rows, double *mu, double *sigma, int ard_dims, bool produce, bool ev);
void launch_batch_eval_full(hipStream_t s, const BatchItem *items, int k, const double *x, const double *Z, double *rows,
                            double *mu, double *sigma, int ard_dims, bool produce, bool ev);
void launch_dinv256_blocks(hipStream_t s, const double *L, int64_t ld, double *Dinv, int nblk);
void launch_diag256_inv_only_ld512(hipStream_t s, const double *L, int64_t ld, double *Dinv);
void launch_convert_block(hipStream_t s, const double *src, int64_t lds_, double *dst, int64_t ldd, int rows,
                          int cols);
void launch_pack_lower(hipStream_t s, const double *in, int64_t n, int64_t npad, double *L,
                       int64_t ld);
void launch_sigma(hipStream_t s, const double *prior, const double *q, int64_t m,
                  double *sigma);
void launch_bwd_panel(hipStream_t s, int64_t rows16, const double *A, int64_t lda, const double *B, int64_t ldb,
                      double *C, int64_t ldc, int64_t ncols, int K, bool tri, bool sub);
int pgrad_slabs(int64_t npad, int64_t m, int *tiles_per_slab);
void launch_pgrad(hipStream_t s, const DevParams *p, int ndim, const double *X, int64_t n, int64_t npad,
                  const double *Z, int64_t m, const double *alpha, const double *Wt, int64_t ld, const double *sigma,
                  double *part, double *dmu, double *dsigma, bool ev);
int pcov_slabs(int64_t npad, int64_t m, int ncu, int *cols_per_slab);
void launch_pcov(hipStream_t s, const DevParams *p, const double *Z, int64_t m, const double *Vt, int64_t ld,
                 int64_t npad, int ncu, double *part, double diag_add, double *out, int64_t mo, int64_t ldo, bool ev);
void launch_pcov_add_mu(hipStream_t s, const double *G, int64_t ldg, const double *mu, int64_t ns, int64_t m, double *out);
int grad_reduce_blocks(int64_t npad);

void launch_grad_reduce(hipStream_t s, const DevParams *p, int ndim, int ard_dims,
                        const double *X, const double *alpha, const double *Kinv, int64_t ld, int64_t n,
                        int64_t npad, double *partials, double *out, bool radial1 = false, int mfma_min_dims = 1,
                        bool ev = false, int max_blocks = 0);
int grad_reduce_blocks_local(int64_t mrows, int64_t ncols);
void launch_grad_reduce_local(hipStream_t s, const DevParams *p, int ndim, int ard_dims,
                              const double *X, const double *alpha, const double *Kinv, int64_t ld,
                              int64_t n, int64_t mrows, int64_t ncols, BlockMap map, double *partials,
                              double *out, bool radial1 = false, int mfma_min_dims = 1, bool ev = false,
                              int max_blocks = 0);
void launch_grad_reduce_local(hipStream_t s, const DevParams *p, int ndim, int ard_dims,
                              const double *X, const double *alpha, const float *Kinv, int64_t ld,
                              int64_t n, int64_t mrows, int64_t ncols, BlockMap map, double *partials,
                              double *out, bool radial1 = false, int mfma_min_dims = 1, bool ev = false,
                              int max_blocks = 0);

void launch_grad_ard_mfma(hipStream_t s, const DevParams *p, int ndim, const double *X, const double *alpha,
                          const double *Kinv, int64_t ld, int64_t n, int nt, int ntc, int ntiles, int blocks,
                          BlockMap map, double *partials);
void launch_grad_ard_mfma(hipStream_t s, const DevParams *p, int ndim, const double *X, const double *alpha,
                          const float *Kinv, int64_t ld, int64_t n, int nt, int ntc, int ntiles, int blocks,
                          BlockMap map, double *partials);

void launch_xgrad(hipStream_t s, const DevParams *p, int ndim, const double *X,
                  const double *alpha, double *Kinv, int64_t ld, int64_t n, int64_t npad,
                  double *gx, bool ev = false);

void launch_rownorm_dot(hipStream_t s, const double *V, int64_t ld, const double *vec,
                        int64_t ncols, int64_t m, double *dot, double *sq);

void launch_zero_upper_blocks(hipStream_t s, double *R, int64_t ld, int64_t npad);
void launch_alpha_from_y(hipStream_t s, const double *Y, int64_t ld, const double *z,
                         int64_t npad, double *alpha);
void launch_zero_block(hipStream_t s, double *B, int64_t ld, int64_t rows, int64_t cols);
void launch_ydiag(hipStream_t s, const double *Dinv, double *Ydiag, int64_t ld);
void launch_tinv_init(hipStream_t s, const double *Dinv, double *X, double *XT, int nsub, int64_t tld);
void launch_tinv_init(hipStream_t s, const float *Dinv, float *X, float *XT, int nsub, int64_t tld);
void launch_blockmm(hipStream_t s, int nprod, const double *const *A, const int64_t *lda, const double *const *B,
                    const int64_t *ldb, double *const *C, const int64_t *ldc, const int *K, double alpha);
void launch_blockmm(hipStream_t s, int nprod, const float *const *A, const int64_t *lda, const float *const *B,
                    const int64_t *ldb, float *const *C, const int64_t *ldc, const int *K, double alpha);
void launch_trace_from_y(hipStream_t s, const float *Y, int64_t ld, int64_t n, int64_t npad, const double *alpha,
                         double *part, double *out);
size_t trsm_small_workspace_bytes(int64_t npad);
void launch_trsm_small(hipStream_t s, const double *L, int64_t ld, const double *Dinv, const double *KsT, int64_t ldk,
                       int64_t npad, int j0, int cnt, void *ws, double *dq, unsigned **tmo_dev);
void launch_trsm_small(hipStream_t s, const float *L, int64_t ld, const float *Dinv, const float *KsT, int64_t ldk,
                       int64_t npad, int j0, int cnt, void *ws, double *dq, unsigned **tmo_dev);
enum { TS_SOL_PAIRED = 0, TS_SOL_COMPACT = 1, TS_SOL_GRANULE = 2, TS_SOL_ROWS = 3 };
struct TsSolution {
  const void *p = nullptr;
  int kind = TS_SOL_PAIRED, width = 32;
};
TsSolution trsm_small_solution(int64_t npad, int j0, int cnt, void *ws, bool f32 = false);
constexpr int APPEND_PART = 64 * 64 + 64;
void launch_append_gram(hipStream_t s, TsSolution v0, TsSolution v1, int m0, int m, int64_t npc, int64_t n,
                        const double *z, double *part, double *Lnew, int64_t ld);
void launch_append_commit(hipStream_t s, const DevParams *p, const double *X2, const double *y2, int m, int64_t n,
                          const double *part, int nslab, double *Lnew, int64_t ld, double *z2out, long long *info,
                          bool ev);
void launch_append_identity_rows(hipStream_t s, double *L, int64_t ld, int64_t r0, int64_t r1, int64_t ncols);
void launch_append_restride(hipStream_t s, const double *src, int64_t ld0, int64_t npad0, double *dst, int64_t ld1,
                            int64_t npad1);
constexpr int REMOVE_W = 32, REMOVE_W_SMALL = 4;
void launch_remove_gather(hipStream_t s, const double *src, int64_t ld0, const int *map, int64_t n1, double *dst,
                          int64_t npad1);
void launch_remove_rows(hipStream_t s, const double *src, const int *map, int64_t n1, int width, double *dst);
void launch_remove_w(hipStream_t s, const double *src, int64_t ld0, const int *map, const int *rem, int mc, int mw, int64_t r0,
                     int64_t n1, int64_t npad1, double *W);
void launch_remove_snap(hipStream_t s, const double *L, int64_t ld, int b0, int nb, double *snap);
void launch_remove_block(hipStream_t s, double *L, int64_t ld, const double *snap, double *W, int mw, int64_t kb, int64_t n1);
void launch_loo_stats(hipStream_t s, const double *Kinv, int64_t ld, const double *alpha, const double *y, int64_t n,
                      int64_t npad, double *mu, double *sigma, double *logp, double *v, double *sc, double *part);
void launch_loo_scale_symv(hipStream_t s, const double *Kinv, int64_t ld, int64_t n, int64_t npad, const double *sc,
                           const double *v, double *B, int64_t ldb, double *upart, double *u);
void launch_loo_rank2(hipStream_t s, double *G, int64_t ld, int64_t n, int64_t npad, const double *u, const double *alpha);
void launch_fill(hipStream_t s, double *p, int64_t count, double v);
void launch_axpy(hipStream_t s, double *a, const double *b, int64_t count);
void launch_dot(hipStream_t s, const double *a, const double *b, int64_t n, double *out);
void launch_transpose_sq(hipStream_t s, const double *src, int64_t lds_, double *dst, int64_t ldd,
                         int n);
void launch_transpose_sq(hipStream_t s, const float *src, int64_t lds_, float *dst, int64_t ldd, int n);
void launch_pack_blocks(hipStream_t s, double *dst, const double *src, int nblk, int64_t blk,
                        int first, int stride);
int64_t chunk_tdot_scratch(int64_t max_rows, int nb);
void launch_chunk_tdot(hipStream_t s, const double *chunk, int64_t rows, int nb, const double *v,
                       double *part, double *out);
void launch_chunk_tdot(hipStream_t s, const float *chunk, int64_t rows, int nb, const double *v,
                       double *part, double *out);
void launch_chunk_alpha(hipStream_t s, const double *Ych, int mloc, int nloc, int nb, BlockMap map,
                        const double *z, double *out);
void launch_chunk_alpha(hipStream_t s, const float *Ych, int mloc, int nloc, int nb, BlockMap map,
                        const double *z, double *out);
void launch_chunk_sumsq(hipStream_t s, const double *Ych, int mloc, int nloc, int nb, BlockMap map, int64_t n, double *part,
                        double *out);
void launch_chunk_sumsq(hipStream_t s, const float *Ych, int mloc, int nloc, int nb, BlockMap map, int64_t n, double *part,
                        double *out);
void launch_logdet_block(hipStream_t s, const double *L, int64_t ld, int64_t row0, int64_t n, int nb,
                         double *acc);
void launch_sumsq_info(hipStream_t s, const double *z, int64_t n, const long long *info, double *out);
void launch_info_to_double(hipStream_t s, const long long *info, double *out);
void launch_extract_lower(hipStream_t s, const double *L, int64_t ld, int64_t n,
                          double *out);

}
```

### gogp_amd/csrc/gemm_plan.h

```cpp
#pragma once
#include <algorithm>

#include "common.h"

namespace gogp {

struct GemmPrecision {
  int kstep;
  bool band_513_768;
  bool cand_batch;
  bool lauum_kbeg0;
};
constexpr int SGEMM_BK = 32;
constexpr GemmPrecision GEMM_F64 = {GEMM_BK, true, true, true}, GEMM_F32 = {SGEMM_BK, false, false, false};

struct GemmPlan {
  int mt, nt, nkt, kend, trap, rule, tpb_shift, rblk0, cblk0, pr, Pr, pc, Pc, beta0, new_row0, ktri, prio, krag0;
  int kbeg0;
  GemmMode mode;
  int ntiles;
  double flops;
  int64_t tag;
  int tile, waves;
  unsigned gridx, gridz;
};

inline GemmPlan gemm_plan(GemmMode mode, int mt, int nt, int64_t K, const GemmGrid *grid, int ncand, GemmPrecision prec) {
  constexpr int NONE = 0x7fffffff;
  GemmPlan p{};
  if (!prec.cand_batch) ncand = 1;
  p.mt = mt;
  p.nt = nt;
  p.nkt = (int)(K / prec.kstep);
  p.kend = (int)K;
  p.trap = mode == GEMM_TRAP;
  p.rule = p.tpb_shift = p.rblk0 = p.cblk0 = p.pr = p.pc = p.beta0 = 0;
  p.Pr = p.Pc = 1;
  p.new_row0 = (mode == GEMM_LOWER && grid && grid->new_row0 >= 0) ? grid->new_row0 : NONE;
  p.ktri = (mode == GEMM_RECT && grid && grid->ktri) ? 1 : 0;
  p.prio = grid ? grid->prio : 0;
  p.krag0 = (mode != GEMM_LAUUM && mode != GEMM_TRAP && grid && grid->krag0 >= 0 && !p.ktri) ? grid->krag0 : NONE;
  p.kbeg0 = (mode == GEMM_LAUUM && grid && prec.lauum_kbeg0) ? grid->kbeg0 : 0;
  if (grid && grid->rule) {
    p.rule = grid->rule;
    p.tpb_shift = grid->tpb_shift;
    p.rblk0 = grid->rblk0;
    p.cblk0 = grid->cblk0;
    p.pr = grid->pr;
    p.Pr = grid->Pr;
    p.pc = grid->pc;
    p.Pc = grid->Pc;
    p.beta0 = grid->beta0;
  }
  int ntiles;
  double flops;
  if (mode == GEMM_TRAP) {
    mode = GEMM_RECT;
    ntiles = mt * nt;
    const int nb = nt / 2;
    flops = 2.0 * TILE * TILE * (double)K * ((double)mt * nt - 4.0 * nb * (nb - 1) / 2.0);
  } else if (mode == GEMM_RECT) {
    ntiles = mt * nt;
    flops = 2.0 * (double)mt * TILE * (double)nt * TILE * (double)K;
    if (p.ktri) {
      flops = 0;
      for (int j = 0; j < nt; ++j)
        flops += 2.0 * (double)mt * TILE * TILE * (double)std::min<int64_t>(K, (int64_t)(j + 1) * TILE);
    }
    if (p.krag0 != NONE) {
      flops = 0;
      for (int i = 0; i < mt; ++i)
        flops += 2.0 * (double)nt * TILE * TILE * (double)(K - (int64_t)std::max(0, i - p.krag0) * TILE);
    }
    if (p.rule) {
      const int tpb = 1 << p.tpb_shift;
      long kept = 0;
      for (int bi = 0; bi < mt / tpb; ++bi)
        for (int bj = 0; bj < nt / tpb; ++bj) {
          const int gI = (p.rblk0 + bi) * p.Pr + p.pr, gJ = (p.cblk0 + bj) * p.Pc + p.pc;
          kept += gI > gJ ? (long)tpb * tpb : (gI == gJ ? (long)tpb * (tpb + 1) / 2 : 0);
        }
      flops = 2.0 * (double)kept * TILE * TILE * (double)K;
    }
  } else {
    ntiles = mt * (mt + 1) / 2;
    if (mode == GEMM_LOWER && p.krag0 != NONE) {
      flops = 0;
      for (int i = 0; i < mt; ++i)
        flops += 2.0 * (double)(i + 1) * TILE * TILE * (double)(K - (int64_t)std::max(0, i - p.krag0) * TILE);
    } else if (mode == GEMM_LOWER) {
      flops = 2.0 * (double)ntiles * TILE * TILE * (double)K;
    } else {
      flops = 0;
      for (int i = 0; i < mt; ++i)
        flops += 2.0 * (double)(i + 1) * TILE * TILE * (double)(K - std::max<int64_t>((int64_t)i * TILE, p.kbeg0));
    }
  }
  p.mode = mode;
  p.ntiles = ntiles;
  p.flops = flops * ncand;
  p.tag = (int64_t)mode * 100000000LL + (int64_t)(K / 16) * 100000LL + (int64_t)std::min(ntiles, 99999);
  const long total_tiles = (long)ntiles * ncand;
  const bool small = (mode != GEMM_LAUUM) && (total_tiles < (grid ? grid->small_below : 384) ||
                                              (prec.band_513_768 && total_tiles > 512 && total_tiles <= 768));
  if (p.prio == 1 && !small) p.prio = 0;
  p.tile = small ? 64 : TILE;
  p.waves = (mode == GEMM_LAUUM || (!small && total_tiles >= 3072)) ? 8 : 4;
  p.gridx = p.rule ? 8 * ((mt + 7) / 8) * nt : ntiles;
  p.gridz = (unsigned)ncand;
  if (small) {
    p.mt = mt * 2;
    p.nt = nt * 2;
    p.tpb_shift += 1;
    if (p.new_row0 != NONE) p.new_row0 *= 2;
    if (p.krag0 != NONE) p.krag0 *= 2;
    p.gridx = (mode == GEMM_RECT) ? (p.rule ? 8 * ((p.mt + 7) / 8) * p.nt : p.mt * p.nt) : p.mt * (p.mt + 1) / 2;
  }
  return p;
}

}
```

### gogp_amd/csrc/gemm_tile.h

```cpp
#pragma once
#include <type_traits>

#include <hip/hip_ext.h>

#include "common.h"
#include "gemm_plan.h"

namespace gogp {

template <class T>
struct GemmArgsCommon {
  const T *A;
  const T *B;
  T *C;
  long lda, ldb, ldc;
  int mt, nt;
  int nkt;
  T alpha, beta;
  int kend;
  int trap;
  int rule, tpb_shift, rblk0, cblk0, pr, Pr, pc, Pc, beta0;
  int new_row0;
  int ktri;
  int prio;
  int krag0;
};
template <class T>
struct GemmArgs : GemmArgsCommon<T> {};
template <>
struct GemmArgs<double> : GemmArgsCommon<double> {
  int kbeg0;
  long bstride;
#ifdef GOGP_WGSTAMP
  unsigned long long *stamps;
#endif
};

template <class T>
__device__ __forceinline__ void load16_to_lds(const T *gsrc, T *lds_wave_base) {
#if defined(__HIP_DEVICE_COMPILE__)
  __builtin_amdgcn_global_load_lds(gsrc, lds_wave_base, 16, 0, 0);
#endif
}
__device__ __forceinline__ void raise_wave_priority() {
#if defined(__HIP_DEVICE_COMPILE__)
  __builtin_amdgcn_s_setprio(3);
#endif
}
__device__ __forceinline__ void wait_vmcnt0() {
#if defined(__HIP_DEVICE_COMPILE__)
  __builtin_amdgcn_s_waitcnt(0x0F70);
#endif
}

__device__ __forceinline__ int xcd_chunk(int t) {
  const int nwg = gridDim.x;
  const int q = nwg >> 3, r = nwg & 7;
  const int xcd = t & 7;
  return (xcd < r ? xcd * (q + 1) : r * (q + 1) + (xcd - r) * q) + (t >> 3);
}

template <int BT, int BK, class T>
__device__ __forceinline__ bool rect_tile_assignment(const GemmArgs<T> &g, int &ti_out, int &tj_out, T &beta_out,
                                                     int &kbeg_out, int &nkt_out) {
  int t = blockIdx.x;
  if (!g.rule) t = xcd_chunk(t);
  int ti, tj;
  if (g.rule) {
    const int x = t & 7, slot = t >> 3;
    const int rr = slot / g.nt;
    ti = x + 8 * rr;
    tj = slot - rr * g.nt;
    if (ti >= g.mt) return false;
  } else {
    ti = t / g.nt;
    tj = t - ti * g.nt;
    if (g.trap && (tj * BT) / PANEL > (ti * BT) / PANEL) return false;
  }
  T beta = g.beta;
  if (g.rule) {
    const int gI = (g.rblk0 + (ti >> g.tpb_shift)) * g.Pr + g.pr;
    const int gJ = (g.cblk0 + (tj >> g.tpb_shift)) * g.Pc + g.pc;
    const int msk = (1 << g.tpb_shift) - 1;
    if (gI < gJ || (gI == gJ && (ti & msk) < (tj & msk))) return false;
    if (g.rule == 2) beta = (gI == g.beta0) ? T(0) : T(1);
  }
  int kbeg = 0, nkt = g.nkt;
  if (g.ktri) nkt = min(nkt, (tj + 1) * BT / BK);
  if (ti > g.krag0) {
    kbeg = (ti - g.krag0) * BT;
    nkt -= kbeg / BK;
  }
  ti_out = ti, tj_out = tj, beta_out = beta, kbeg_out = kbeg, nkt_out = nkt;
  return true;
}

template <class T>
struct TileKernel;

template <class T>
void launch_tile_gemm(hipStream_t s, GemmMode mode, int mt, int nt, int64_t K, double alpha, const T *A, int64_t lda,
                      const T *B, int64_t ldb, double beta, T *C, int64_t ldc, GemmProfile *prof, const GemmGrid *grid) {
  if (mt <= 0 || nt <= 0 || K <= 0) return;
  constexpr bool F64 = std::is_same_v<T, double>;
  const GemmPlan p = gemm_plan(mode, mt, nt, K, grid, tl_batch.k, F64 ? GEMM_F64 : GEMM_F32);
  GemmArgs<T> g;
  g.A = A;
  g.B = B;
  g.C = C;
  g.lda = lda;
  g.ldb = ldb;
  g.ldc = ldc;
  g.alpha = (T)alpha;
  g.beta = (T)beta;
  g.mt = p.mt, g.nt = p.nt, g.nkt = p.nkt, g.kend = p.kend, g.trap = p.trap;
  g.rule = p.rule, g.tpb_shift = p.tpb_shift, g.rblk0 = p.rblk0, g.cblk0 = p.cblk0, g.beta0 = p.beta0;
  g.pr = p.pr, g.Pr = p.Pr, g.pc = p.pc, g.Pc = p.Pc;
  g.new_row0 = p.new_row0, g.ktri = p.ktri, g.prio = p.prio, g.krag0 = p.krag0;
  if constexpr (F64) {
    g.kbeg0 = p.kbeg0;
    g.bstride = tl_batch.stride;
#ifdef GOGP_WGSTAMP
    const int shape = p.tile == 64 ? 1 : (p.waves == 8 ? 3 : 2);
    g.stamps = stamp_reserve((long long)p.gridx * p.gridz, 10000000000LL * shape + p.tag, s);
#endif
  }
  hipEvent_t e0 = nullptr, e1 = nullptr;
  if (prof && prof->on) {
    if (prof->used + 2 > prof->pool.size()) {
      size_t old = prof->pool.size();
      prof->pool.resize(old + 1024);
      for (size_t i = old; i < prof->pool.size(); ++i) (void)hipEventCreate(&prof->pool[i]);
    }
    e0 = prof->pool[prof->used++];
    e1 = prof->pool[prof->used++];
    prof->flops += p.flops;
    prof->launches += 1;
    prof->lflops.push_back(p.flops);
    prof->ltag.push_back(p.tag);
  }
  using K_ = TileKernel<T>;
  void (*kernel)(GemmArgs<T>);
  if (p.tile == 64)
    kernel = p.mode == GEMM_RECT ? K_::template get<GEMM_RECT, 64, 4>() : K_::template get<GEMM_LOWER, 64, 4>();
  else if (p.waves == 4)
    kernel = p.mode == GEMM_RECT ? K_::template get<GEMM_RECT, 128, 4>() : K_::template get<GEMM_LOWER, 128, 4>();
  else
    kernel = p.mode == GEMM_RECT    ? K_::template get<GEMM_RECT, 128, 8>()
             : p.mode == GEMM_LOWER ? K_::template get<GEMM_LOWER, 128, 8>()
                                    : K_::template get<GEMM_LAUUM, 128, 8>();
  const dim3 gridd(p.gridx, 1, p.gridz), block(p.waves * 64);
  if (e0)
    hipExtLaunchKernelGGL(kernel, gridd, block, 0, s, e0, e1, 0, g);
  else
    GOGP_KLAUNCH(kernel, gridd, block, 0, s, g);
}

}
```

### gogp_amd/csrc/handle.h

```cpp
#pragma once
#include <algorithm>
#include <array>
#include <string>
#include <vector>

#include "common.h"

namespace gogp {
struct Dist2D;
}
using gogp::DevParams;
using gogp::GemmProfile;

constexpr int REFINE_SLABS = 8;

constexpr int HS_INFO = 8;
constexpr int HS_TRACE = 9;
constexpr int HS_TMO = 10;
constexpr int HS_PIVOT = 12;
constexpr int HS_GRAD = 16;
static_assert(HS_INFO < HS_TMO && HS_TMO < HS_PIVOT && HS_PIVOT < HS_GRAD, "the staging words lie below the gradient's sums");
static_assert(HS_GRAD + gogp::NACC == gogp::BATCH_ROW, "the pinned row is a batch row");

struct EvalBufs {
  DevParams *devP = nullptr;
  long long *info = nullptr;
  double *scalars = nullptr;
  double *gout = nullptr;
  double *bufA = nullptr, *bufL = nullptr, *bufY = nullptr, *Dinv = nullptr;
  double *z = nullptr, *w = nullptr, *alpha = nullptr;
  double *gpart = nullptr;
};

struct NBufs {
  double *dX = nullptr, *dy = nullptr, *bufA = nullptr, *bufL = nullptr, *Dinv = nullptr;
  double *z = nullptr, *w = nullptr, *alpha = nullptr, *gpart = nullptr;
};

struct gogp_handle;
struct Workspace {
  void *p = nullptr;
  size_t bytes = 0;
  inline int reserve(gogp_handle *h, size_t need);
  void release() {
    (void)hipFree(p);
    p = nullptr;
    bytes = 0;
  }
  template <class T>
  T *as() const { return static_cast<T *>(p); }
};

struct EvalState {
  bool factored = false, have_alpha = false, have_kinv = false;
  bool observed = false, with_obs = false;
  bool grad_valid = false;
  bool trtri_done = false;
  double lml = 0.0;
  double cond_lb = 1.0;
  int64_t notpd = -1;
};

struct CandGraphKey {
  int k = 0;
  int64_t n = 0, cap_npad = 0;
  size_t stride = 0;
  const void *arena = nullptr, *dX = nullptr, *dy = nullptr, *hostP = nullptr, *hscal = nullptr;
  bool operator==(const CandGraphKey &o) const {
    return k == o.k && n == o.n && cap_npad == o.cap_npad && stride == o.stride && arena == o.arena && dX == o.dX &&
           dy == o.dy && hostP == o.hostP && hscal == o.hscal;
  }
};

struct gogp_handle : EvalBufs, EvalState {
  gogp_desc desc;
  int device = 0;
  int ns = 0, nn = 0, P = 0, D = 0;
  int ard_dims = 0;
  bool radial1 = false;
  int nevents = 0, ev_axis = 0;
  double events[GOGP_MAX_EVENTS][3] = {};
  bool ev() const { return nevents > 0; }
  int64_t n = 0, npad = 0;
  int nblk = 0;
  double *dX = nullptr, *dy = nullptr;
  double *dscr = nullptr;
  double *D64 = nullptr;
  int64_t cap_d64 = 0;
  int diag_fp64 = 1;
  bool d64_active = false;
  int prec = 64;
  size_t esz() const { return prec == 32 ? sizeof(float) : sizeof(double); }
  int refine_steps = 1;
  double *rw = nullptr, *rz = nullptr, *rd = nullptr, *rpart = nullptr;
  DevParams *hostP = nullptr;
  double *hscal = nullptr;
  int64_t cap_npad = 0;
  int64_t cap_y = 0;
  double *dZ = nullptr, *KsT = nullptr, *Vt = nullptr, *pvec = nullptr;
  int64_t cap_m = 0, cap_mp_npad = 0;
  Workspace pg_ws;
  Workspace pc_ws;
  int ncu = 0;
  hipStream_t s = nullptr;
  hipStream_t sp = nullptr;
  char *cand_arena = nullptr;
  size_t cand_stride = 0;
  int cand_cap_k = 0;
  int64_t cand_cap_npad = 0;
  DevParams *cand_hostP = nullptr;
  double *cand_hscal = nullptr;
  int cand_host_k = 0;
  int batch_k = 1;
  bool batch_mode = false;
  int use_graph = 1;
  bool graph_failed = false;
  int graph_nodes = 0;
  std::string graph_note;
  hipGraphExec_t cand_graph = nullptr;
  hipStream_t sg = nullptr;
  CandGraphKey cand_graph_key, cand_seen_key;
  double *bt_X = nullptr, *bt_y = nullptr;
  int64_t bt_rows = 0, bt_cap_rows = 0;
  std::vector<int64_t> bt_off, bt_n;
  bool bt_have = false;
  char *bt_din = nullptr, *bt_hin = nullptr;
  size_t bt_in_cap = 0;
  double *bt_dout = nullptr, *bt_hout = nullptr;
  size_t bt_out_cap = 0;
  gogp::Dist2D *dist = nullptr;
  hipStream_t sl = nullptr;
  hipStream_t s2 = nullptr;
  hipStream_t st = nullptr;
  hipStream_t sk = nullptr;
  void *stream_set = nullptr;
  std::vector<hipEvent_t> evs;
  int lookahead = 1;
  int superpanel = 2;
  int eager = 1;
  int superpanel_head = -1;
  int head_remaining = 16;
  int chain_prio = -1;
  int tiny = 1;
  int chain_slabs = 0;
  int chain_split = -1;
  int ktri = 1;
  double *TX = nullptr, *Tmt = nullptr;
  int64_t tinv_ld = 0;
  size_t cap_tinv = 0;
  int grad_prec = 64;
  float *g32A = nullptr, *g32L = nullptr, *g32Y = nullptr, *g32D = nullptr;
  int64_t g32_cap = 0;
  int produce_panels = 4;
  int produce_small_below = 1024;
  int produce_tinv = 1;
  bool tinv_valid = false, tinv_pending = false;
  int64_t tinv_sig = 0;
  int produce_small_max = 64;
  Workspace small_ws;
  int produce_groups = 2;
  int krag = 1;
  int ard_mfma_min = 1;
  int kinv_split = 60;
  int64_t kinv_c1 = 0;
  int kinv_fused = -1;
  bool kinv_pending = false;
  bool trtri_pending = false;
  bool ydone_valid = false;
  bool alpha_pending = false;
  std::vector<double> theta_s, theta_n;
  bool have_data = false;
  bool have_theta = false;
  bool z_valid = false;
  Workspace app_ws;
  Workspace rm_ws;
  Workspace loo_vec;
  Workspace loo_mat;
  double yta = 0.0;
  int trace_fp64 = 1;
  double cond_limit = 1e16;
  std::vector<double> grad_cache;
  std::string err;
  GemmProfile prof;
  std::vector<hipEvent_t> aux_ev[GOGP_PROF_NCLASS];
  size_t aux_used[GOGP_PROF_NCLASS] = {0, 0, 0, 0};
};

struct AuxTimer {
  gogp_handle *h;
  int cls;
  hipStream_t s;
  hipEvent_t e1 = nullptr;
  AuxTimer(gogp_handle *h_, int cls_, hipStream_t s_) : h(h_), cls(cls_), s(s_) {
    if (!h->prof.on || cls < 0 || cls >= GOGP_PROF_NCLASS) return;
    auto &pool = h->aux_ev[cls];
    size_t &used = h->aux_used[cls];
    while (pool.size() < used + 2) {
      hipEvent_t e = nullptr;
      (void)hipEventCreate(&e);
      pool.push_back(e);
    }
    (void)hipEventRecord(pool[used], s);
    e1 = pool[used + 1];
    used += 2;
  }
  ~AuxTimer() {
    if (e1) (void)hipEventRecord(e1, s);
  }
};

#define HIPCHK(h, call)                                                                \
  do {                                                                                 \
    hipError_t e_ = (call);                                                            \
    if (e_ != hipSuccess) {                                                            \
      char buf_[512];                                                                  \
      snprintf(buf_, sizeof buf_, "%s failed: %s (%s:%d)", #call, hipGetErrorString(e_), \
               __FILE__, __LINE__);                                                    \
      (h)->err = buf_;                                                                 \
      (void)hipGetLastError();  \
      return (e_ == hipErrorOutOfMemory) ? GOGP_ENOMEM : GOGP_EHIP;                     \
    }                                                                                  \
  } while (0)

inline int Workspace::reserve(gogp_handle *h, size_t need) {
  if (p && bytes >= need) return GOGP_OK;
  release();
  HIPCHK(h, hipMalloc(&p, need));
  bytes = need;
  return GOGP_OK;
}

static inline unsigned *hs_tmo(const gogp_handle *h) { return reinterpret_cast<unsigned *>(h->hscal + HS_TMO); }

static inline void nbufs_free(const NBufs &b) {
  for (double *q : {b.dX, b.dy, b.bufA, b.bufL, b.Dinv, b.z, b.w, b.alpha, b.gpart}) (void)hipFree(q);
}
static inline hipError_t nbufs_alloc(const gogp_handle *h, int64_t cap, NBufs *b) {
  const size_t nn = (size_t)cap * (size_t)cap * h->esz(), vec = (size_t)cap * sizeof(double);
  hipError_t e = hipMalloc(&b->dX, ((size_t)cap * h->D + GOGP_MAX_NDIM) * sizeof(double));
  if (e == hipSuccess) e = hipMalloc(&b->dy, vec);
  if (e == hipSuccess) e = hipMalloc(&b->bufA, nn);
  if (e == hipSuccess) e = hipMalloc(&b->bufL, nn);
  if (e == hipSuccess) e = hipMalloc(&b->Dinv, (size_t)(cap / gogp::PANEL) * gogp::PANEL * gogp::PANEL * h->esz());
  if (e == hipSuccess) e = hipMalloc(&b->z, vec);
  if (e == hipSuccess) e = hipMalloc(&b->w, vec);
// ... 58 lines not shown
```

### gogp_amd/csrc/solve.hip

```cpp
#include "common.h"

namespace gogp {

__device__ __forceinline__ void load8(const double *p, double *o) {
  const double2 *q = reinterpret_cast<const double2 *>(p);
  const double2 a = q[0], b = q[1], c = q[2], d = q[3];
  o[0] = a.x; o[1] = a.y; o[2] = b.x; o[3] = b.y; o[4] = c.x; o[5] = c.y; o[6] = d.x; o[7] = d.y;
}
__device__ __forceinline__ void load8(const float *p, double *o) {
  const float4 *q = reinterpret_cast<const float4 *>(p);
  const float4 a = q[0], b = q[1];
  o[0] = a.x; o[1] = a.y; o[2] = a.z; o[3] = a.w; o[4] = b.x; o[5] = b.y; o[6] = b.z; o[7] = b.w;
}
__device__ __forceinline__ void load2(const double *p, double &a, double &b) {
  const double2 v = *reinterpret_cast<const double2 *>(p);
  a = v.x;
  b = v.y;
}
__device__ __forceinline__ void load2(const float *p, double &a, double &b) {
  const float2 v = *reinterpret_cast<const float2 *>(p);
  a = v.x;
  b = v.y;
}
__device__ __forceinline__ void store2zero(double *p) {
// ... 261 lines not shown
    red[1][wid] = b;
  }
  __syncthreads();
  if (threadIdx.x == 0) {
    if (dot) dot[j] = red[0][0] + red[0][1] + red[0][2] + red[0][3];
    if (sq) sq[j] = red[1][0] + red[1][1] + red[1][2] + red[1][3];
  }
}

void launch_rownorm_dot(hipStream_t s, const double *V, int64_t ld, const double *vec,
                        int64_t ncols, int64_t m, double *dot, double *sq) {
  if (m <= 0) return;
  GOGP_KLAUNCH(rownorm_dot_kernel<double>, dim3((unsigned)m), dim3(256), 0, s, V, (long)ld, vec,
                     (long)ncols, dot, sq);
}
void launch_rownorm_dot(hipStream_t s, const float *V, int64_t ld, const double *vec,
                        int64_t ncols, int64_t m, double *dot, double *sq) {
  if (m <= 0) return;
  GOGP_KLAUNCH(rownorm_dot_kernel<float>, dim3((unsigned)m), dim3(256), 0, s, V, (long)ld, vec,
                     (long)ncols, dot, sq);
}

template <class T>
__global__ __launch_bounds__(256) void trace_rows_kernel(const T *__restrict__ Y, long ld, long ncols,
                                                         const double *__restrict__ alpha, double *__restrict__ part) {
  __shared__ double red[4];
  const long i = blockIdx.x;
  const long q0 = (i / PANEL) * PANEL;
  const T *row = Y + i * ld;
  double b = 0.0;
  for (long q = q0 + threadIdx.x; q < ncols; q += 256) {
    const double v = (double)row[q];
    b += v * v;
  }
  b = wave_sum(b);
  if ((threadIdx.x & 63) == 0) red[threadIdx.x >> 6] = b;
  __syncthreads();
  if (threadIdx.x == 0) part[i] = alpha[i] * alpha[i] - ((red[0] + red[1]) + (red[2] + red[3]));
}
__global__ __launch_bounds__(1024) void sum_kernel(const double *__restrict__ v, long n, double *__restrict__ out) {
  __shared__ double red[16];
  double a = 0.0;
  for (long i = threadIdx.x; i < n; i += 1024) a += v[i];
  a = wave_sum(a);
  if ((threadIdx.x & 63) == 0) red[threadIdx.x >> 6] = a;
  __syncthreads();
  if (threadIdx.x == 0) {
    double t = 0.0;
    for (int w = 0; w < 16; ++w) t += red[w];
    out[0] = t;
  }
}
void launch_trace_from_y(hipStream_t s, const float *Y, int64_t ld, int64_t n, int64_t npad, const double *alpha,
                         double *part, double *out) {
  if (n <= 0) return;
  GOGP_KLAUNCH(trace_rows_kernel<float>, dim3((unsigned)n), dim3(256), 0, s, Y, (long)ld, (long)npad, alpha, part);
  GOGP_KLAUNCH(sum_kernel, dim3(1), dim3(1024), 0, s, (const double *)part, (long)n, out);
}

template <class T>
__global__ __launch_bounds__(256) void zero_upper_kernel(T *__restrict__ R, long ld,
                                                         long npad, long bstride) {
  R = cand(R, bstride);
  const long row = blockIdx.y;
  const long cstart = (row / PANEL + 1) * PANEL;
  const long c = cstart + ((long)blockIdx.x * 256 + threadIdx.x) * 2;
  if (c >= npad) return;
  store2zero(R + row * ld + c);
}

void launch_zero_upper_blocks(hipStream_t s, double *R, int64_t ld, int64_t npad) {
  if (npad <= PANEL) return;
  dim3 grid((unsigned)((npad / 2 + 255) / 256), (unsigned)(npad - PANEL), (unsigned)tl_batch.k);
  GOGP_KLAUNCH(zero_upper_kernel<double>, grid, dim3(256), 0, s, R, (long)ld, (long)npad,
                     tl_batch.stride);
}
void launch_zero_upper_blocks(hipStream_t s, float *R, int64_t ld, int64_t npad) {
  if (npad <= PANEL) return;
  dim3 grid((unsigned)((npad / 2 + 255) / 256), (unsigned)(npad - PANEL));
  GOGP_KLAUNCH(zero_upper_kernel<float>, grid, dim3(256), 0, s, R, (long)ld, (long)npad, 0L);
}

template <class T>
__global__ __launch_bounds__(256) void ydiag_kernel(const T *__restrict__ Dinv,
                                                    T *__restrict__ Y, long ld, long bstride) {
  Dinv = cand(Dinv, bstride);
  Y = cand(Y, bstride);
  __shared__ T tile[32][33];
  const int bx = blockIdx.x & 7, by = blockIdx.x >> 3;
  const int tx = threadIdx.x & 31, ty = threadIdx.x >> 5;
#pragma unroll
  for (int r = 0; r < 32; r += 8) tile[ty + r][tx] = Dinv[(by * 32 + ty + r) * 256 + bx * 32 + tx];
  __syncthreads();
#pragma unroll
  for (int r = 0; r < 32; r += 8) Y[(long)(bx * 32 + ty + r) * ld + by * 32 + tx] = tile[tx][ty + r];
}

void launch_ydiag(hipStream_t s, const double *Dinv, double *Ydiag, int64_t ld) {
  GOGP_KLAUNCH(ydiag_kernel<double>, dim3(64, 1, (unsigned)tl_batch.k), dim3(256), 0, s, Dinv, Ydiag,
                     (long)ld, tl_batch.stride);
}
void launch_ydiag(hipStream_t s, const float *Dinv, float *Ydiag, int64_t ld) {
  GOGP_KLAUNCH(ydiag_kernel<float>, dim3(64), dim3(256), 0, s, Dinv, Ydiag, (long)ld, 0L);
}

template <class T>
__global__ __launch_bounds__(256) void tinv_init_kernel(const T *__restrict__ Dinv, T *__restrict__ X,
                                                        T *__restrict__ XT, int nsub, long tld, long bstride) {
  Dinv = cand(Dinv, bstride);
  X = cand(X, bstride);
  if (XT) XT = cand(XT, bstride);
  __shared__ T tile[32][33];
  const int tpr = nsub * 8;
  const int bx = blockIdx.x % tpr, by = blockIdx.x / tpr;
  const int I = by >> 3, J = bx >> 3;
  const int tx = threadIdx.x & 31, ty = threadIdx.x >> 5;
  const long r0 = (long)by * 32, c0 = (long)bx * 32;
  if (I == J) {
    const T *D = Dinv + (long)I * 256 * 256 + (long)(by & 7) * 32 * 256 + (bx & 7) * 32;
#pragma unroll
    for (int r = 0; r < 32; r += 8) {
      const T v = D[(ty + r) * 256 + tx];
      X[(r0 + ty + r) * tld + c0 + tx] = v;
      tile[ty + r][tx] = v;
    }
    if (XT) {
      __syncthreads();
      const long tr0 = (long)I * 256 + (long)(bx & 7) * 32, tc0 = (long)I * 256 + (long)(by & 7) * 32;
#pragma unroll
      for (int r = 0; r < 32; r += 8) XT[(tr0 + ty + r) * tld + tc0 + tx] = tile[tx][ty + r];
    }
  } else if (I < J) {
#pragma unroll
    for (int r = 0; r < 32; r += 8) X[(r0 + ty + r) * tld + c0 + tx] = (T)0;
  } else if (XT) {
#pragma unroll
    for (int r = 0; r < 32; r += 8) XT[(r0 + ty + r) * tld + c0 + tx] = (T)0;
  }
}
void launch_tinv_init(hipStream_t s, const double *Dinv, double *X, double *XT, int nsub, int64_t tld) {
  GOGP_KLAUNCH(tinv_init_kernel<double>, dim3(nsub * 8 * nsub * 8, 1, (unsigned)tl_batch.k), dim3(256), 0, s, Dinv,
                     X, XT, nsub, (long)tld, tl_batch.stride);
}
void launch_tinv_init(hipStream_t s, const float *Dinv, float *X, float *XT, int nsub, int64_t tld) {
  GOGP_KLAUNCH(tinv_init_kernel<float>, dim3(nsub * 8 * nsub * 8), dim3(256), 0, s, Dinv, X, XT, nsub, (long)tld, 0L);
}

constexpr int BLOCKMM_MAX = 6;
template <class T>
struct BlockMM {
  const T *A[BLOCKMM_MAX];
  const T *B[BLOCKMM_MAX];
  T *C[BLOCKMM_MAX];
  long lda[BLOCKMM_MAX], ldb[BLOCKMM_MAX], ldc[BLOCKMM_MAX];
  int K[BLOCKMM_MAX];
  double alpha;
  long bstride;
};
typedef double bmm_f64x4 __attribute__((ext_vector_type(4)));
template <class T>
__global__ __launch_bounds__(256, 2) void blockmm_kernel(BlockMM<T> g) {
  constexpr int KC = 32, AS = KC + 1, BS = 64 + 2;
  __shared__ double As[64 * AS];
  __shared__ double Bs[KC * BS];
  const int b = blockIdx.y;
  const T *A = cand(g.A[b], g.bstride);
  const T *B = cand(g.B[b], g.bstride);
  T *C = cand(g.C[b], g.bstride);
  const long lda = g.lda[b], ldb = g.ldb[b], ldc = g.ldc[b];
  const int K = g.K[b];
  const int tid = threadIdx.x, lane = tid & 63, w = tid >> 6;
  const int tr = blockIdx.x >> 2, tc = blockIdx.x & 3;
  A += (long)tr * 64 * lda;
  B += tc * 64;
  C += (long)tr * 64 * ldc + tc * 64;
  const int ar = tid >> 2, ak = (tid & 3) * 8, bk = tid >> 3, bc = (tid & 7) * 8;
  double ra[8], rb[8];
  auto gload = [&](int k0) {
#pragma unroll
    for (int i = 0; i < 8; ++i) ra[i] = (double)A[(long)ar * lda + k0 + ak + i];
#pragma unroll
    for (int i = 0; i < 8; ++i) rb[i] = (double)B[(long)(k0 + bk) * ldb + bc + i];
  };
  bmm_f64x4 acc[4];
#pragma unroll
  for (int n = 0; n < 4; ++n) acc[n] = (bmm_f64x4){0.0, 0.0, 0.0, 0.0};
// ... 436 lines not shown
```

### gogp_amd/csrc/testhooks.hip

```cpp
#include <cstdlib>
#include <cstring>
#include <stdio.h>

#include "common.h"
#include "gemm_plan.h"
#include "../../include/gogp_testhooks.h"

struct gogp_handle;
namespace gogp {
int dist_init_replay(gogp_handle *h, int rank, int nranks, int prow, int pcol);
}
extern "C" int gogp_test_dist_init_replay(void *h, int rank, int nranks, int prow, int pcol) {
  return gogp::dist_init_replay(static_cast<gogp_handle *>(h), rank, nranks, prow, pcol);
}

namespace gogp_th {
void launch_diag256(hipStream_t s, const double *A, int64_t ld, double *Lout, int64_t ldl,
                    double *Dinv, int64_t row0, int64_t nvalid, long long *info);
void launch_diag256_stamped(hipStream_t s, const double *A, double *Lout, double *Dinv,
                            long long *info, unsigned long long *stamps);
void launch_panel128_stamped(hipStream_t s, const double *A, double *Lout, int64_t rows_below, long long *info,
                             unsigned long long *stamps);
}

// ... 122 lines not shown
  if (hipEventSynchronize(e1) != hipSuccess) return GOGP_EHIP;
  float ms = 0;
  (void)hipEventElapsedTime(&ms, e0, e1);
  const double flops = (double)blocks * 4.0 * (double)iters * 8.0 * 2.0 * 16 * 16 * 4;
  *tflops = flops / (ms * 1e-3) / 1e12;
  unsigned long long h[2] = {0, 0};
  (void)hipMemcpy(h, clk, 16, hipMemcpyDeviceToHost);
  if (cyc_per_mfma) *cyc_per_mfma = (double)h[0] / ((double)iters * 8.0 * 2.0);
  if (clock_mhz) *clock_mhz = h[1] ? (double)h[0] / (double)h[1] * 100.0 : 0.0;
  (void)hipEventDestroy(e0);
  (void)hipEventDestroy(e1);
  (void)hipFree(sink);
  (void)hipFree(clk);
  return GOGP_OK;
}


}

using namespace gogp;

extern "C" int gogp_mfma_f64_peak(int device, int iters, double *tflops, double *cyc_per_mfma,
                                  double *clock_mhz) {
  if (!tflops || iters <= 0) return GOGP_EARG;
  int ndev = 0;
  if (hipGetDeviceCount(&ndev) != hipSuccess || ndev <= 0) return GOGP_EHIP;
  if (device >= 0 && hipSetDevice(device) != hipSuccess) return GOGP_EHIP;
  return mfma_f64_peak(iters, tflops, cyc_per_mfma, clock_mhz);
}

extern "C" int gogp_mfma_f32_peak(int device, int iters, double *tflops, double *cyc_per_mfma,
                                  double *clock_mhz) {
  if (!tflops || iters <= 0) return GOGP_EARG;
  int ndev = 0;
  if (hipGetDeviceCount(&ndev) != hipSuccess || ndev <= 0) return GOGP_EHIP;
  if (device >= 0 && hipSetDevice(device) != hipSuccess) return GOGP_EHIP;
  return mfma_f32_peak(iters, tflops, cyc_per_mfma, clock_mhz);
}

extern "C" int gogp_test_dgemm_nt(int device, int64_t M, int64_t N, int64_t K, double alpha,
                                  const double *A, const double *B, double beta, double *C) {
  if (!A || !B || !C || M <= 0 || N <= 0 || K <= 0) return GOGP_EARG;
  if (M % TILE || N % TILE || K % GEMM_BK) return GOGP_EARG;
  int ndev = 0;
  if (hipGetDeviceCount(&ndev) != hipSuccess || ndev <= 0) return GOGP_EHIP;
  if (device >= 0 && hipSetDevice(device) != hipSuccess) return GOGP_EHIP;
  double *dA = nullptr, *dB = nullptr, *dC = nullptr;
  hipError_t e = hipMalloc(&dA, (size_t)M * K * sizeof(double));
  if (e == hipSuccess) e = hipMalloc(&dB, (size_t)N * K * sizeof(double));
  if (e == hipSuccess) e = hipMalloc(&dC, (size_t)M * N * sizeof(double));
  if (e == hipSuccess) e = hipMemcpy(dA, A, (size_t)M * K * sizeof(double), hipMemcpyHostToDevice);
  if (e == hipSuccess) e = hipMemcpy(dB, B, (size_t)N * K * sizeof(double), hipMemcpyHostToDevice);
  if (e == hipSuccess) e = hipMemcpy(dC, C, (size_t)M * N * sizeof(double), hipMemcpyHostToDevice);
  if (e == hipSuccess) {
    launch_dgemm_nt(0, GEMM_RECT, (int)(M / TILE), (int)(N / TILE), K, alpha, dA, K, dB, K, beta,
                    dC, N, nullptr);
    e = hipDeviceSynchronize();
  }
  if (e == hipSuccess) e = hipMemcpy(C, dC, (size_t)M * N * sizeof(double), hipMemcpyDeviceToHost);
  (void)hipFree(dA);
  (void)hipFree(dB);
  (void)hipFree(dC);
  return e == hipSuccess ? GOGP_OK : GOGP_EHIP;
}

namespace {
bool covers(int64_t len, int64_t off, int64_t ld, int64_t rows, int64_t cols, int64_t k, int64_t stride) {
  if (len <= 0 || off < 0 || ld < cols || rows <= 0 || cols <= 0 || k <= 0 || stride < 0) return false;
  const int64_t hi = off + (k - 1) * stride + (rows - 1) * ld + cols;
  return hi <= len;
}
bool device_ok(int device) {
  int ndev = 0;
  if (hipGetDeviceCount(&ndev) != hipSuccess || ndev <= 0) return false;
  return device < 0 || hipSetDevice(device) == hipSuccess;
}
bool gemm_launch_args_ok(int precision, int mode, int mt, int nt, int64_t K, const gogp_test_gemm_opts &o) {
  if (precision != 64 && precision != 32) return false;
  if (mode < GEMM_RECT || mode > GEMM_TRAP || mt <= 0 || nt <= 0 || K <= 0) return false;
  const int64_t kstep = precision == 64 ? GEMM_BK : SGEMM_BK, al = 16 / (precision / 8);
  if (K % kstep || K > (1 << 30)) return false;
  if ((mode == GEMM_LOWER || mode == GEMM_LAUUM) && mt != nt) return false;
  if (o.k < 1 || o.k > 64 || o.bstride < 0 || o.bstride % al || (o.k > 1 && o.bstride == 0)) return false;
  if (precision == 32 && (o.k > 1 || o.kbeg0 != 0)) return false;
  if (o.kbeg0 < 0 || o.kbeg0 % kstep || o.kbeg0 > K || (o.kbeg0 && mode != GEMM_LAUUM)) return false;
  if (o.new_row0 < -1 || (o.new_row0 >= 0 && mode != GEMM_LOWER)) return false;
  if (o.ktri && mode != GEMM_RECT) return false;
  if (o.krag0 < -1 || (o.krag0 >= 0 && (o.ktri || (mode != GEMM_RECT && mode != GEMM_LOWER)))) return false;
  if (o.krag0 >= 0 && o.krag0 < mt && K < (int64_t)(mt - o.krag0) * TILE) return false;
  if (o.rule < 0 || o.rule > 2 || (o.rule && mode != GEMM_RECT)) return false;
  if (o.rule && (o.tpb_shift < 0 || o.tpb_shift > 8 || o.rblk0 < 0 || o.cblk0 < 0 || o.Pr < 1 || o.Pc < 1 ||
                 o.pr < 0 || o.pr >= o.Pr || o.pc < 0 || o.pc >= o.Pc))
    return false;
  return true;
}
const gogp_test_gemm_opts GEMM_OPTS_DEFAULT = {0, -1, -1, 0, 384, 0, 0, 0, 0, 0, 0, 1, 0, 1, -1, 1, 0};
GemmGrid gemm_grid_of(const gogp_test_gemm_opts &o) {
  GemmGrid g;
  g.ktri = o.ktri;
  g.krag0 = o.krag0;
  g.new_row0 = o.new_row0;
  g.kbeg0 = o.kbeg0;
  g.small_below = o.small_below;
  g.prio = o.prio;
  g.rule = o.rule;
  g.tpb_shift = o.tpb_shift;
  g.rblk0 = o.rblk0;
  g.cblk0 = o.cblk0;
  g.pr = o.pr;
  g.Pr = o.Pr;
  g.pc = o.pc;
  g.Pc = o.Pc;
  g.beta0 = o.beta0;
  return g;
}
}

extern "C" int gogp_test_gemm_plan(int precision, int mode, int mt, int nt, int64_t K, const gogp_test_gemm_opts *opt,
                                   gogp_test_gemm_plan_out *out) {
  const gogp_test_gemm_opts o = opt ? *opt : GEMM_OPTS_DEFAULT;
  if (!out || !gemm_launch_args_ok(precision, mode, mt, nt, K, o)) return GOGP_EARG;
  const GemmGrid g = gemm_grid_of(o);
  const GemmPlan p = gemm_plan((GemmMode)mode, mt, nt, K, &g, o.k, precision == 64 ? GEMM_F64 : GEMM_F32);
  out->tile = p.tile;
  out->waves = p.waves;
  out->grid_x = p.gridx;
  out->grid_z = p.gridz;
  out->flops = p.flops;
  out->tag = p.tag;
  return GOGP_OK;
}

extern "C" int gogp_test_gemm_nt(int device, int precision, int mode, int mt, int nt, int64_t K, double alpha,
                                 double beta, const void *A, int64_t a_len, int64_t a_off, int64_t lda, const void *B,
                                 int64_t b_len, int64_t b_off, int64_t ldb, void *C, int64_t c_len, int64_t c_off,
                                 int64_t ldc, const gogp_test_gemm_opts *opt) {
  const gogp_test_gemm_opts o = opt ? *opt : GEMM_OPTS_DEFAULT;
  if (!A || !B || !C || !gemm_launch_args_ok(precision, mode, mt, nt, K, o)) return GOGP_EARG;
  const int64_t es = precision / 8, al = 16 / es;
  if (alpha == 0.0 || (precision == 32 && (float)alpha == 0.0f)) return GOGP_EARG;
  if (lda % al || ldb % al || ldc % al || a_off % al || b_off % al || c_off % al) return GOGP_EARG;
  const int64_t M = (int64_t)mt * TILE, N = (int64_t)nt * TILE;
  if (!covers(a_len, a_off, lda, M, K, o.k, o.bstride) || !covers(b_len, b_off, ldb, N, K, o.k, o.bstride) ||
      !covers(c_len, c_off, ldc, M, N, o.k, o.bstride))
    return GOGP_EARG;
  if (!device_ok(device)) return GOGP_EHIP;

  char *dA = nullptr, *dB = nullptr, *dC = nullptr;
  hipError_t e = hipMalloc(&dA, (size_t)(a_len * es));
  if (e == hipSuccess) e = hipMalloc(&dB, (size_t)(b_len * es));
  if (e == hipSuccess) e = hipMalloc(&dC, (size_t)(c_len * es));
  if (e == hipSuccess) e = hipMemcpy(dA, A, (size_t)(a_len * es), hipMemcpyHostToDevice);
  if (e == hipSuccess) e = hipMemcpy(dB, B, (size_t)(b_len * es), hipMemcpyHostToDevice);
  if (e == hipSuccess) e = hipMemcpy(dC, C, (size_t)(c_len * es), hipMemcpyHostToDevice);
  if (e == hipSuccess) {
    const GemmGrid g = gemm_grid_of(o);
    tl_batch.k = o.k;
    tl_batch.stride = (long)(o.bstride * es);
    if (precision == 64)
      launch_gemm_nt(0, (GemmMode)mode, mt, nt, K, alpha, (const double *)dA + a_off, lda, (const double *)dB + b_off, ldb,
                     beta, (double *)dC + c_off, ldc, nullptr, &g);
    else
      launch_gemm_nt(0, (GemmMode)mode, mt, nt, K, alpha, (const float *)dA + a_off, lda, (const float *)dB + b_off, ldb,
                     beta, (float *)dC + c_off, ldc, nullptr, &g);
    tl_batch.k = 1;
    tl_batch.stride = 0;
    e = hipGetLastError();
    if (e == hipSuccess) e = hipDeviceSynchronize();
  }
  if (e == hipSuccess) e = hipMemcpy(C, dC, (size_t)(c_len * es), hipMemcpyDeviceToHost);
  (void)hipFree(dA);
  (void)hipFree(dB);
  (void)hipFree(dC);
  return e == hipSuccess ? GOGP_OK : GOGP_EHIP;
}

extern "C" int gogp_test_diag_syrk(int device, int bs, const float *L, int64_t l_len, int64_t l_off, int64_t ld,
                                   int64_t K, int64_t row_stride, double *D64, int64_t d_len, int nblocks) {
  if (!L || !D64 || (bs != PANEL && bs != 2 * PANEL) || nblocks < 1 || nblocks > 4096) return GOGP_EARG;
  if (K < 16 || K % 16 || ld % 4 || l_off % 4 || row_stride % 4) return GOGP_EARG;
  if (bs == PANEL && row_stride != PANEL * ld) return GOGP_EARG;
  if (!covers(l_len, l_off, ld, bs, K, nblocks, row_stride) || d_len < (int64_t)nblocks * bs * bs) return GOGP_EARG;
// ... 744 lines not shown
```

### include/gogp_testhooks.h

```cpp
#ifndef GOGP_TESTHOOKS_H
#define GOGP_TESTHOOKS_H

#include <stdint.h>

#include "gogp_hip.h"

#ifdef __cplusplus
extern "C" {
#endif

int gogp_mfma_f64_peak(int device, int iters, double *tflops, double *cyc_per_mfma,
                       double *clock_mhz);
int gogp_mfma_f32_peak(int device, int iters, double *tflops, double *cyc_per_mfma,
                       double *clock_mhz);

int gogp_test_dgemm_nt(int device, int64_t M, int64_t N, int64_t K, double alpha,
                       const double *A, const double *B, double beta, double *C);

typedef struct gogp_test_gemm_opts {
  int32_t ktri, krag0, new_row0, kbeg0, small_below, prio;
  int32_t rule, tpb_shift, rblk0, cblk0, pr, Pr, pc, Pc, beta0;
  int32_t k;
  int64_t bstride;
} gogp_test_gemm_opts;

int gogp_test_gemm_nt(int device, int precision, int mode, int mt, int nt, int64_t K, double alpha, double beta,
                      const void *A, int64_t a_len, int64_t a_off, int64_t lda, const void *B, int64_t b_len,
                      int64_t b_off, int64_t ldb, void *C, int64_t c_len, int64_t c_off, int64_t ldc,
                      const gogp_test_gemm_opts *opt);

typedef struct gogp_test_gemm_plan_out {
  int32_t tile, waves;
  int64_t grid_x, grid_z;
  double flops;
  int64_t tag;
} gogp_test_gemm_plan_out;
int gogp_test_gemm_plan(int precision, int mode, int mt, int nt, int64_t K, const gogp_test_gemm_opts *opt,
                        gogp_test_gemm_plan_out *out);

int gogp_test_diag_syrk(int device, int bs, const float *L, int64_t l_len, int64_t l_off, int64_t ld, int64_t K,
                        int64_t row_stride, double *D64, int64_t d_len, int nblocks);

int gogp_test_diag256_product(int device, int variant, const double *A, int64_t ld, double *L, int64_t ldl,
                              double *Dinv, int64_t row0, int64_t nvalid, long long *info);


int64_t gogp_test_trsm_small_workspace(int64_t npad);

int gogp_test_trsm_small(int device, int precision, int64_t npad, const void *L, int64_t l_len, int64_t ld,
                         const void *Dinv, const void *KsT, int64_t k_len, int64_t ldk, int j0, int cnt, double *dq,
                         int64_t dq_len, void *sol, int64_t sol_len, int *kind, int *width, int64_t *sol_off,
                         unsigned *tmo);

int gogp_test_trsv_steps(int device, int precision, int dir, int64_t npad, const void *L, int64_t l_len, int64_t ld,
                         const void *Dinv, int b0, int b1, int k, int64_t bstride, double *w, int64_t w_len, double *out,
                         int64_t out_len);

int gogp_test_alpha_from_y(int device, int precision, int64_t npad, const void *Y, int64_t y_len, int64_t ld,
                           const double *z, int64_t z_len, double *alpha, int64_t alpha_len);

int gogp_test_rownorm_dot(int device, int precision, const void *V, int64_t v_len, int64_t ld, int64_t ncols, int64_t m,
                          const double *vec, int64_t vec_len, double *dot, int64_t dot_len, double *sq, int64_t sq_len);

int gogp_test_tinv(int device, int precision, int nsub, const void *Dinv, void *X, int64_t x_len, int64_t tld, int with_xt,
                   void *XT);

int gogp_test_blockmm(int device, int precision, int nprod, void *arena, int64_t arena_len, const int64_t *a_off,
                      const int64_t *lda, const int64_t *b_off, const int64_t *ldb, const int64_t *c_off,
                      const int64_t *ldc, const int *K, double alpha, int k, int64_t bstride);


typedef struct gogp_test_kparams {
  int32_t ndim, nterms;
  int32_t kind[GOGP_MAX_TERMS], ard[GOGP_MAX_TERMS];
  double c[GOGP_MAX_TERMS], w[GOGP_MAX_TERMS], inv_len[GOGP_MAX_TERMS][GOGP_MAX_NDIM];
  double noise_var, dnoise;
  int32_t nevents, ev_axis;
  double ev_from[GOGP_MAX_EVENTS], ev_to[GOGP_MAX_EVENTS], ev_disc[GOGP_MAX_EVENTS];
} gogp_test_kparams;

#define GOGP_TEST_NACC (16 + GOGP_MAX_NDIM)

int gogp_test_grad_blocks(int64_t npad, int64_t mrows, int64_t ncols, int max_blocks);

int gogp_test_grad_reduce(int device, int precision, const gogp_test_kparams *kparams, int ard_dims, int radial1,
                          int mfma_min, int ev, const double *X, int64_t x_len, const double *alpha, int64_t alpha_len,
                          const void *Kinv, int64_t kinv_len, int64_t ld, int64_t n, int64_t npad, int max_blocks, int k,
                          int64_t bstride, double *partials, int64_t partials_len, double *out);

int gogp_test_grad_reduce_local(int device, int precision, const gogp_test_kparams *kparams, int ard_dims, int radial1,
                                int mfma_min, int ev, const double *X, int64_t x_len, const double *alpha,
                                int64_t alpha_len, const void *Kinv, int64_t kinv_len, int64_t ld, int64_t n, int64_t npad,
                                int64_t mrows, int64_t ncols, int nb_shift, int pr, int Pr, int pc, int Pc, int max_blocks,
                                int k, int64_t bstride, double *partials, int64_t partials_len, double *out);

int gogp_test_xgrad(int device, const gogp_test_kparams *kparams, int ev, const double *X, int64_t x_len,
                    const double *alpha, int64_t alpha_len, double *Kinv, int64_t kinv_len, int64_t ld, int64_t n,
                    int64_t npad, double *gx, int64_t gx_len);

int gogp_bench_gemm(int device, int mode, int mt, int nt, int64_t K, int reps,
                    double *ms_per_launch, double *tflops);

int gogp_test_diag256(int device, const double *A, double *Lout, double *Dinv,
                      unsigned long long *stamps, double *elapsed_us);

int gogp_test_valu_cost(int device, double *out8);
// ... 14 lines not shown
```

Before: 13.74.

## Add tail-split triangular inverse path and fuse ydiag with zero-block launch

Adds an optional trailing region of the fp64 triangular inverse, selected by an `inv_tail` knob. There, rows above the tail cut are filled by a separate GEMM against a transposed copy of the tail block, using a new `ktri0` offset so the triangular-K GEMM can start at an interior tile. This needs a new XT buffer and a transpose kernel, and the candidate-batch arena layout grows to hold it. Separately, the diagonal Dinv copy and the zeroing of the block below it are merged into one kernel launch to cut launch count per panel. The tail path is off by default because `inv_tail` defaults to -1; only the launch fusion runs without tuning.

```diff
diff --git a/gogp_amd/_lib.py b/gogp_amd/_lib.py
--- a/gogp_amd/_lib.py
+++ b/gogp_amd/_lib.py
@@ -33,9 +33,9 @@
 class CGemmOpts(ctypes.Structure):
     _fields_ = [(n, ctypes.c_int32) for n in ("ktri", "krag0", "new_row0", "kbeg0", "small_below", "prio", "rule",
                                               "tpb_shift", "rblk0", "cblk0", "pr", "Pr", "pc", "Pc", "beta0", "k")]
-    _fields_ += [("bstride", ctypes.c_int64)]
+    _fields_ += [("bstride", ctypes.c_int64), ("ktri0", ctypes.c_int32)]
     DEFAULTS = dict(ktri=0, krag0=-1, new_row0=-1, kbeg0=0, small_below=384, prio=0, rule=0, tpb_shift=0, rblk0=0,
-                    cblk0=0, pr=0, Pr=1, pc=0, Pc=1, beta0=-1, k=1, bstride=0)
+                    cblk0=0, pr=0, Pr=1, pc=0, Pc=1, beta0=-1, k=1, bstride=0, ktri0=0)
 
 
 class CKParams(ctypes.Structure):
diff --git a/gogp_amd/csrc/api.hip b/gogp_amd/csrc/api.hip
--- a/gogp_amd/csrc/api.hip
+++ b/gogp_amd/csrc/api.hip
@@ -74,7 +74,9 @@
   nbufs_free(nbufs_of(h));
   nbufs_put(h, NBufs());
   (void)hipFree(h->bufY);
-  h->bufY = nullptr;
+  (void)hipFree(h->bufXT);
+  h->bufY = h->bufXT = nullptr;
+  h->cap_xt = 0;
   (void)hipFree(h->rw);
   (void)hipFree(h->rz);
   (void)hipFree(h->rd);
@@ -118,6 +120,7 @@
   h->cand_stride = 0;
   h->cand_cap_k = h->cand_host_k = 0;
   h->cand_cap_npad = 0;
+  h->cand_cap_xt = 0;
 }
 
 static void free_m_buffers(gogp_handle *h) {
@@ -445,6 +448,15 @@
   h->cap_y = cap;
   return GOGP_OK;
 }
+static int ensure_xt(gogp_handle *h, int64_t width) {
+  if (width <= h->cap_xt) return GOGP_OK;
+  (void)hipFree(h->bufXT);
+  h->bufXT = nullptr;
+  h->cap_xt = 0;
+  HIPCHK(h, hipMalloc(&h->bufXT, (size_t)width * (size_t)width * h->esz()));
+  h->cap_xt = width;
+  return GOGP_OK;
+}
 
 static int ensure_d64(gogp_handle *h) {
   if (h->D64 && h->cap_d64 >= h->npad) return GOGP_OK;
@@ -581,6 +593,23 @@
 static inline InnerGroup inner_group(int q, int64_t c2, int64_t CE) {
   const int done = q + 1, grp = done & -done;
   return {grp, c2 - (int64_t)grp * PANEL, std::min(c2 + (int64_t)grp * PANEL, CE)};
+}
+
+static int64_t inv_tail_start(const gogp_handle *h) {
+  const int64_t npad = h->npad;
+  const int t = h->inv_tail < 0 ? 0 : h->inv_tail;
+  if (t == 0 || h->prec != 64 || h->dist || h->grad_prec == 32) return npad;
+  int64_t lo = std::max<int64_t>(0, npad - (int64_t)t * PANEL);
+  const std::vector<SuperPanel> sps = superpanels(h);
+  if (h->kinv_split > 0)
+    for (const SuperPanel &P : sps)
+      if (P.CE() < npad && P.CE() * 100 >= npad * (int64_t)h->kinv_split) {
+        lo = std::max(lo, P.CE());
+        break;
+      }
+  for (const SuperPanel &P : sps)
+    if (P.C0() >= lo) return P.C0() > 0 ? P.C0() : npad;
+  return npad;
 }
 
 constexpr int TMT_BLOCKS = 8;
@@ -647,54 +676,70 @@
 struct InvBufs {
   T *A, *Y;
   const T *L, *Dinv;
+  T *XT = nullptr;
 };
 template <class T>
-static void trtri_superstep(gogp_handle *h, const InvBufs<T> &B, const SuperPanel &P, hipStream_t st, hipStream_t s2) {
+static void trtri_superstep(gogp_handle *h, const InvBufs<T> &B, const SuperPanel &P, hipStream_t st, hipStream_t s2,
+                            int64_t CT) {
   const int64_t npad = h->npad, ld = npad;
   T *R = B.A, *Y = B.Y;
   const T *L = B.L;
   GemmProfile *pf = &h->prof;
   const int P0 = P.P0;
   const int64_t C0 = P.C0(), CE = P.CE();
+  const bool tail = C0 >= CT;
+  const int64_t r0 = tail ? CT : 0;
+  T *Rr = R + r0 * ld, *Yr = Y + r0 * ld;
   for (int q = 0; q < P.nsub; ++q) {
     const int p = P0 + q;
     const int64_t c0 = (int64_t)p * PANEL, c2 = c0 + PANEL;
     const T *Dp = B.Dinv + (size_t)p * PANEL * PANEL;
-    launch_ydiag(st, Dp, Y + c0 * ld + c0, ld);
-    if (c2 < CE)
-      launch_zero_block(st, Y + c2 * ld + c0, ld, CE - c2, PANEL);
-    if (c0 > 0) {
+    launch_ydiag_zero(st, Dp, Y + c0 * ld + c0, ld, CE - c2);
+    if (c0 > r0) {
       GemmGrid gtri = chain_grid(h);
       gtri.ktri = h->ktri;
-      launch_gemm_nt(st, GEMM_RECT, (int)(c0 / TILE), 2, PANEL, 1.0, R + c0, ld, Dp, PANEL, 0.0,
-                      Y + c0, ld, pf, &gtri);
+      launch_gemm_nt(st, GEMM_RECT, (int)((c0 - r0) / TILE), 2, PANEL, 1.0, Rr + c0, ld, Dp, PANEL, 0.0,
+                      Yr + c0, ld, pf, &gtri);
     }
     if (c2 < CE) {
       const InnerGroup g = inner_group(q, c2, CE);
       GemmGrid gch = chain_grid(h);
-      if (h->krag) gch.krag0 = (int)(g.k0 / TILE);
-      launch_gemm_nt(st, GEMM_RECT, (int)(c2 / TILE), (int)((g.ce - c2) / TILE), (int64_t)g.grp * PANEL,
-                      -1.0, Y + g.k0, ld, L + c2 * ld + g.k0, ld, 1.0, R + c2, ld, pf, &gch);
+      if (h->krag) gch.krag0 = (int)((g.k0 - r0) / TILE);
+      launch_gemm_nt(st, GEMM_RECT, (int)((c2 - r0) / TILE), (int)((g.ce - c2) / TILE), (int64_t)g.grp * PANEL,
+                      -1.0, Yr + g.k0, ld, L + c2 * ld + g.k0, ld, 1.0, Rr + c2, ld, pf, &gch);
     }
   }
   order(h, EV_BASE + 4 * P0 + 2, st, s2);
   const int nt = (int)((npad - CE) / TILE);
   if (nt > 0) {
     const int64_t Kw = CE - C0;
-    const int mr = (int)(CE / TILE);
+    const int mr = (int)((CE - r0) / TILE);
     const int ntn = nt < 2 * P.next_nsub ? nt : 2 * P.next_nsub;
     if (P0 > 0 && st != s2)
       (void)gogp::rec_stream_wait(st, ev(h, EV_BASE + 4 * P.prevP0 + 3));
     GemmGrid gch = chain_grid(h), gbulk;
-    if (h->krag) gch.krag0 = gbulk.krag0 = (int)(C0 / TILE);
-    launch_gemm_nt(st, GEMM_RECT, mr, ntn, Kw, -1.0, Y + C0, ld, L + CE * ld + C0, ld, 1.0,
-                    R + CE, ld, pf, &gch);
+    if (h->krag) gch.krag0 = gbulk.krag0 = (int)((C0 - r0) / TILE);
+    launch_gemm_nt(st, GEMM_RECT, mr, ntn, Kw, -1.0, Yr + C0, ld, L + CE * ld + C0, ld, 1.0,
+                    Rr + CE, ld, pf, &gch);
     if (nt > ntn) {
       const int64_t C3 = CE + (int64_t)ntn * TILE;
-      launch_gemm_nt(s2, GEMM_RECT, mr, nt - ntn, Kw, -1.0, Y + C0, ld, L + C3 * ld + C0, ld, 1.0,
-                      R + C3, ld, pf, &gbulk);
+      launch_gemm_nt(s2, GEMM_RECT, mr, nt - ntn, Kw, -1.0, Yr + C0, ld, L + C3 * ld + C0, ld, 1.0,
+                      Rr + C3, ld, pf, &gbulk);
     }
     (void)gogp::rec_event_record(ev(h, EV_BASE + 4 * P0 + 3), s2);
+  }
+  if constexpr (std::is_same_v<T, double>) {
+    if (tail) {
+      const int64_t WT = npad - CT;
+      T *X = B.XT + (C0 - CT) * WT;
+      launch_xt_rows(s2, Y + CT * ld + C0, ld, X, WT, CE - C0, CE - CT, WT);
+      GemmGrid gx;
+      gx.ktri = h->ktri;
+      gx.ktri0 = (int)((C0 - CT) / TILE);
+      launch_gemm_nt(s2, GEMM_RECT, (int)(CT / TILE), (int)((CE - C0) / TILE), CE - CT, 1.0, R + CT, ld, X, WT, 0.0,
+                      Y + C0, ld, pf, &gx);
+      if (CE == npad && st != s2) order(h, EV_BASE + 4 * P0 + 3, s2, st);
+    }
   }
 }
 
@@ -724,7 +769,7 @@
   launch_convert_block(st, h->Dinv + (size_t)P.P0 * PANEL * PANEL, PANEL, h->g32D + (size_t)P.P0 * PANEL * PANEL, PANEL,
                        (int)W, PANEL);
   const InvBufs<float> B{h->g32A, h->g32Y, h->g32L, h->g32D};
-  trtri_superstep<float>(h, B, P, st, s2);
+  trtri_superstep<float>(h, B, P, st, s2, h->npad);
 }
 
 template <class T>
@@ -744,16 +789,20 @@
   else
     launch_zero_upper_blocks(s, reinterpret_cast<T *>(h->bufA), h->npad, h->npad);
 }
+static int inverse_tail_of(gogp_handle *h, bool fp32, bool mixed, bool fuse_kinv, int64_t *CT) {
+  *CT = (fp32 || mixed || fuse_kinv) ? h->npad : inv_tail_start(h);
+  return ensure_xt(h, h->npad - *CT);
+}
 template <class T>
 static void inverse_superstep(gogp_handle *h, bool mixed, const SuperPanel &P, hipStream_t st, hipStream_t s2,
-                              bool fuse_kinv) {
+                              bool fuse_kinv, int64_t CT) {
   if (mixed) {
     mixed_superstep(h, P, st, s2);
     if (fuse_kinv) kinv_accumulate<float>(h, h->g32Y, h->g32A, P.C0(), P.CE());
   } else {
     const InvBufs<T> B{reinterpret_cast<T *>(h->bufA), reinterpret_cast<T *>(h->bufY), reinterpret_cast<const T *>(h->bufL),
-                       reinterpret_cast<const T *>(h->Dinv)};
-    trtri_superstep<T>(h, B, P, st, s2);
+                       reinterpret_cast<const T *>(h->Dinv), reinterpret_cast<T *>(h->bufXT)};
+    trtri_superstep<T>(h, B, P, st, s2, CT);
     if (fuse_kinv) kinv_accumulate<T>(h, B.Y, B.A, P.C0(), P.CE());
   }
 }
@@ -822,6 +871,7 @@
   bool mixed = !fp32 && mixed_gradient(h);
   bool fuse_kinv = eager && (h->kinv_fused < 0 ? (npad <= 10240 || mixed) : h->kinv_fused != 0);
   int split = fp32 ? 0 : chain_split_of(h, eager);
+  int64_t CT = h->npad;
 
   void d64_init(hipStream_t q, int first, int nblk) const {
     if constexpr (fp32)
@@ -927,7 +977,7 @@
   void inverse_behind(const SuperPanel &P) const {
     const int64_t CE = P.CE();
     (void)gogp::rec_stream_wait(st, ev(h, EV_BASE + 4 * P.P0));
-    inverse_superstep<T>(h, mixed, P, st, s2, fuse_kinv);
+    inverse_superstep<T>(h, mixed, P, st, s2, fuse_kinv, CT);
     if (!fp32 && !fuse_kinv && !mixed && !h->batch_mode && h->kinv_split > 0 && h->kinv_c1 == 0 && CE < npad &&
         CE * 100 >= npad * (int64_t)h->kinv_split) {
       (void)gogp::rec_stream_wait(h->sk, ev(h, EV_BASE + 4 * P.P0 + 2));
@@ -971,10 +1021,11 @@
 
 template <class T>
 static int factorize_t(gogp_handle *h, bool eager) {
-  const Sweep<T> c{h, eager && h->lookahead != 0};
+  Sweep<T> c{h, eager && h->lookahead != 0};
   begin_evaluation(h, {c.s, c.sp});
   int rc = gogp_upload_params(h);
   if (rc == GOGP_OK && (c.mixed || c.eager)) rc = c.mixed ? ensure_g32(h) : ensure_y(h);
+  if (rc == GOGP_OK && c.eager) rc = inverse_tail_of(h, c.fp32, c.mixed, c.fuse_kinv, &c.CT);
   if (rc == GOGP_OK) rc = c.build_gram();
   if (rc != GOGP_OK) return rc;
   if (c.fp32) HIPCHK(h, hipMemsetAsync(h->scalars + 5, 0, sizeof(double), c.sp));
@@ -1153,7 +1204,10 @@
     if (rcy != GOGP_OK) return rcy;
     zero_inverse_rhs<T>(h, mixed, s);
     order(h, EV_INIT, s, sp);
-    for (const SuperPanel &P : superpanels(h)) inverse_superstep<T>(h, mixed, P, sp, s, false);
+    int64_t CT = npad;
+    const int rct = inverse_tail_of(h, sizeof(T) == 4, mixed, false, &CT);
+    if (rct != GOGP_OK) return rct;
+    for (const SuperPanel &P : superpanels(h)) inverse_superstep<T>(h, mixed, P, sp, s, false, CT);
     order(h, EV_TRTRI, sp, s);
     h->trtri_done = true;
   } else if (h->trtri_pending) {
@@ -1427,7 +1481,7 @@
 constexpr int64_t GRAPH_MAX_NPAD = 1024;
 constexpr int64_t GRAPH_EXPLICIT_MAX_NPAD = 8192;
 
-static EvalBufs cand_layout(char *base, int64_t npad, size_t esz, size_t *bytes = nullptr) {
+static EvalBufs cand_layout(char *base, int64_t npad, int64_t xt, size_t esz, size_t *bytes = nullptr) {
   EvalBufs b;
   size_t o = 0;
   auto take = [&](auto *&p, size_t n) {
@@ -1447,6 +1501,7 @@
   take(b.bufA, nn);
   take(b.bufL, nn);
   take(b.bufY, nn);
+  if (xt > 0) take(b.bufXT, (size_t)xt * (size_t)xt * esz);
   if (bytes) *bytes = align_up(o, 4096);
   return b;
 }
@@ -1463,19 +1518,22 @@
     HIPCHK(h, hipHostMalloc((void **)&h->cand_hscal, (size_t)k * BATCH_ROW * sizeof(double), hipHostMallocDefault));
     h->cand_host_k = k;
   }
-  if (k > h->cand_cap_k || h->npad > h->cand_cap_npad) {
+  const int64_t xt = h->npad - inv_tail_start(h);
+  if (k > h->cand_cap_k || h->npad > h->cand_cap_npad || xt > h->cand_cap_xt) {
     drop_cand_graph(h);
     (void)hipFree(h->cand_arena);
     h->cand_arena = nullptr;
     h->cand_cap_k = 0;
+    const int64_t cap = std::max(h->npad, h->cand_cap_npad), cap_xt = std::max(xt, h->cand_cap_xt);
     h->cand_cap_npad = 0;
-    const int64_t cap = std::max(h->npad, h->cand_cap_npad);
+    h->cand_cap_xt = 0;
     size_t stride = 0;
-    (void)cand_layout(nullptr, cap, h->esz(), &stride);
+    (void)cand_layout(nullptr, cap, cap_xt, h->esz(), &stride);
     HIPCHK(h, hipMalloc((void **)&h->cand_arena, stride * (size_t)k));
     h->cand_stride = stride;
     h->cand_cap_k = k;
     h->cand_cap_npad = cap;
+    h->cand_cap_xt = cap_xt;
   }
   return GOGP_OK;
 }
@@ -1547,10 +1605,11 @@
   const EvalBufs saved_bufs = *h;
   const EvalState saved_state = *h;
   double *const saved_hscal = h->hscal;
-  const int64_t saved_cap_y = h->cap_y;
-  static_cast<EvalBufs &>(*h) = cand_layout(h->cand_arena, h->cand_cap_npad, h->esz());
+  const int64_t saved_cap_y = h->cap_y, saved_cap_xt = h->cap_xt;
+  static_cast<EvalBufs &>(*h) = cand_layout(h->cand_arena, h->cand_cap_npad, h->cand_cap_xt, h->esz());
   h->hscal = h->cand_hscal;
   h->cap_y = h->cand_cap_npad;
+  h->cap_xt = h->cand_cap_xt;
   h->with_obs = false;
   h->batch_k = k;
   h->batch_mode = true;
@@ -1668,6 +1727,7 @@
   static_cast<EvalState &>(*h) = saved_state;
   h->hscal = saved_hscal;
   h->cap_y = saved_cap_y;
+  h->cap_xt = saved_cap_xt;
   h->trtri_pending = h->alpha_pending = h->kinv_pending = false;
   if (first != GOGP_OK && rc == GOGP_OK) h->err = first_msg;
   return first;
@@ -2875,6 +2935,11 @@
     h->kinv_split = (int)value;
     return GOGP_OK;
   }
+  if (strcmp(name, "inv_tail") == 0) {
+    if (value < -1 || value > 4096) return fail(h, GOGP_EARG, "inv_tail must be -1..4096");
+    h->inv_tail = (int)value;
+    return GOGP_OK;
+  }
   if (strcmp(name, "kinv_fused") == 0) {
     h->kinv_fused = value < 0 ? -1 : (value != 0);
     return GOGP_OK;
diff --git a/gogp_amd/csrc/common.h b/gogp_amd/csrc/common.h
--- a/gogp_amd/csrc/common.h
+++ b/gogp_amd/csrc/common.h
@@ -55,6 +55,7 @@
   int rule = 0, tpb_shift = 0, rblk0 = 0, cblk0 = 0, pr = 0, Pr = 1, pc = 0, Pc = 1, beta0 = -1;
   int new_row0 = -1;
   int ktri = 0;
+  int ktri0 = 0;
   int prio = 0;
   int krag0 = -1;
   int small_below = 384;
@@ -115,7 +116,7 @@
                         int64_t m, double *dot, double *sq);
 void launch_zero_upper_blocks(hipStream_t s, float *R, int64_t ld, int64_t npad);
 void launch_zero_block(hipStream_t s, float *B, int64_t ld, int64_t rows, int64_t cols);
-void launch_ydiag(hipStream_t s, const float *Dinv, float *Ydiag, int64_t ld);
+void launch_ydiag_zero(hipStream_t s, const float *Dinv, float *Ydiag, int64_t ld, int64_t rows_below);
 void launch_extract_lower(hipStream_t s, const float *L, int64_t ld, int64_t n, double *out);
 void launch_pack_lower(hipStream_t s, const double *in, int64_t n, int64_t npad, float *L, int64_t ld);
 void launch_convert_block(hipStream_t s, const float *src, int64_t lds_, double *dst, int64_t ldd, int rows,
@@ -235,7 +236,9 @@
 void launch_alpha_from_y(hipStream_t s, const double *Y, int64_t ld, const double *z,
                          int64_t npad, double *alpha);
 void launch_zero_block(hipStream_t s, double *B, int64_t ld, int64_t rows, int64_t cols);
-void launch_ydiag(hipStream_t s, const double *Dinv, double *Ydiag, int64_t ld);
+void launch_ydiag_zero(hipStream_t s, const double *Dinv, double *Ydiag, int64_t ld, int64_t rows_below);
+void launch_xt_rows(hipStream_t s, const double *Y, int64_t ld, double *X, int64_t ldx, int64_t rows, int64_t kcols,
+                    int64_t xcols);
 void launch_tinv_init(hipStream_t s, const double *Dinv, double *X, double *XT, int nsub, int64_t tld);
 void launch_tinv_init(hipStream_t s, const float *Dinv, float *X, float *XT, int nsub, int64_t tld);
 void launch_blockmm(hipStream_t s, int nprod, const double *const *A, const int64_t *lda, const double *const *B,
diff --git a/gogp_amd/csrc/gemm_plan.h b/gogp_amd/csrc/gemm_plan.h
--- a/gogp_amd/csrc/gemm_plan.h
+++ b/gogp_amd/csrc/gemm_plan.h
@@ -10,13 +10,14 @@
   bool band_513_768;
   bool cand_batch;
   bool lauum_kbeg0;
+  bool ktri_origin;
 };
 constexpr int SGEMM_BK = 32;
-constexpr GemmPrecision GEMM_F64 = {GEMM_BK, true, true, true}, GEMM_F32 = {SGEMM_BK, false, false, false};
+constexpr GemmPrecision GEMM_F64 = {GEMM_BK, true, true, true, true}, GEMM_F32 = {SGEMM_BK, false, false, false, false};
 
 struct GemmPlan {
   int mt, nt, nkt, kend, trap, rule, tpb_shift, rblk0, cblk0, pr, Pr, pc, Pc, beta0, new_row0, ktri, prio, krag0;
-  int kbeg0;
+  int kbeg0, ktri0;
   GemmMode mode;
   int ntiles;
   double flops;
@@ -38,6 +39,7 @@
   p.Pr = p.Pc = 1;
   p.new_row0 = (mode == GEMM_LOWER && grid && grid->new_row0 >= 0) ? grid->new_row0 : NONE;
   p.ktri = (mode == GEMM_RECT && grid && grid->ktri) ? 1 : 0;
+  p.ktri0 = (p.ktri && prec.ktri_origin) ? grid->ktri0 : 0;
   p.prio = grid ? grid->prio : 0;
   p.krag0 = (mode != GEMM_LAUUM && mode != GEMM_TRAP && grid && grid->krag0 >= 0 && !p.ktri) ? grid->krag0 : NONE;
   p.kbeg0 = (mode == GEMM_LAUUM && grid && prec.lauum_kbeg0) ? grid->kbeg0 : 0;
@@ -65,7 +67,7 @@
     if (p.ktri) {
       flops = 0;
       for (int j = 0; j < nt; ++j)
-        flops += 2.0 * (double)mt * TILE * TILE * (double)std::min<int64_t>(K, (int64_t)(j + 1) * TILE);
+        flops += 2.0 * (double)mt * TILE * TILE * (double)std::min<int64_t>(K, (int64_t)(p.ktri0 + j + 1) * TILE);
     }
     if (p.krag0 != NONE) {
       flops = 0;
@@ -113,6 +115,7 @@
     p.nt = nt * 2;
     p.tpb_shift += 1;
     if (p.new_row0 != NONE) p.new_row0 *= 2;
+    p.ktri0 *= 2;
     if (p.krag0 != NONE) p.krag0 *= 2;
     p.gridx = (mode == GEMM_RECT) ? (p.rule ? 8 * ((p.mt + 7) / 8) * p.nt : p.mt * p.nt) : p.mt * (p.mt + 1) / 2;
   }
diff --git a/gogp_amd/csrc/gemm_tile.h b/gogp_amd/csrc/gemm_tile.h
--- a/gogp_amd/csrc/gemm_tile.h
+++ b/gogp_amd/csrc/gemm_tile.h
@@ -30,6 +30,7 @@
 template <>
 struct GemmArgs<double> : GemmArgsCommon<double> {
   int kbeg0;
+  int ktri0;
   long bstride;
 #ifdef GOGP_WGSTAMP
   unsigned long long *stamps;
@@ -86,7 +87,11 @@
     if (g.rule == 2) beta = (gI == g.beta0) ? T(0) : T(1);
   }
   int kbeg = 0, nkt = g.nkt;
-  if (g.ktri) nkt = min(nkt, (tj + 1) * BT / BK);
+  if (g.ktri) {
+    int tcol = tj + 1;
+    if constexpr (std::is_same_v<T, double>) tcol += g.ktri0;
+    nkt = min(nkt, tcol * BT / BK);
+  }
   if (ti > g.krag0) {
     kbeg = (ti - g.krag0) * BT;
     nkt -= kbeg / BK;
@@ -119,6 +124,7 @@
   g.new_row0 = p.new_row0, g.ktri = p.ktri, g.prio = p.prio, g.krag0 = p.krag0;
   if constexpr (F64) {
     g.kbeg0 = p.kbeg0;
+    g.ktri0 = p.ktri0;
     g.bstride = tl_batch.stride;
 #ifdef GOGP_WGSTAMP
     const int shape = p.tile == 64 ? 1 : (p.waves == 8 ? 3 : 2);
diff --git a/gogp_amd/csrc/handle.h b/gogp_amd/csrc/handle.h
--- a/gogp_amd/csrc/handle.h
+++ b/gogp_amd/csrc/handle.h
@@ -30,6 +30,7 @@
   double *bufA = nullptr, *bufL = nullptr, *bufY = nullptr, *Dinv = nullptr;
   double *z = nullptr, *w = nullptr, *alpha = nullptr;
   double *gpart = nullptr;
+  double *bufXT = nullptr;
 };
 
 struct NBufs {
@@ -97,6 +98,7 @@
   double *hscal = nullptr;
   int64_t cap_npad = 0;
   int64_t cap_y = 0;
+  int64_t cap_xt = 0;
   double *dZ = nullptr, *KsT = nullptr, *Vt = nullptr, *pvec = nullptr;
   int64_t cap_m = 0, cap_mp_npad = 0;
   Workspace pg_ws;
@@ -108,6 +110,7 @@
   size_t cand_stride = 0;
   int cand_cap_k = 0;
   int64_t cand_cap_npad = 0;
+  int64_t cand_cap_xt = 0;
   DevParams *cand_hostP = nullptr;
   double *cand_hscal = nullptr;
   int cand_host_k = 0;
@@ -161,6 +164,7 @@
   int produce_groups = 2;
   int krag = 1;
   int ard_mfma_min = 1;
+  int inv_tail = -1;
   int kinv_split = 60;
   int64_t kinv_c1 = 0;
   int kinv_fused = -1;
diff --git a/gogp_amd/csrc/solve.hip b/gogp_amd/csrc/solve.hip
--- a/gogp_amd/csrc/solve.hip
+++ b/gogp_amd/csrc/solve.hip
@@ -367,10 +367,15 @@
 }
 
 template <class T>
-__global__ __launch_bounds__(256) void ydiag_kernel(const T *__restrict__ Dinv,
-                                                    T *__restrict__ Y, long ld, long bstride) {
+__global__ __launch_bounds__(256) void ydiag_zero_kernel(const T *__restrict__ Dinv, T *__restrict__ Y, long ld,
+                                                         long bstride) {
   Dinv = cand(Dinv, bstride);
   Y = cand(Y, bstride);
+  if (blockIdx.x >= 64) {
+    const long r = 256 + 2 * (long)(blockIdx.x - 64) + (threadIdx.x >> 7);
+    store2zero(Y + r * ld + 2 * (threadIdx.x & 127));
+    return;
+  }
   __shared__ T tile[32][33];
   const int bx = blockIdx.x & 7, by = blockIdx.x >> 3;
   const int tx = threadIdx.x & 31, ty = threadIdx.x >> 5;
@@ -380,13 +385,39 @@
 #pragma unroll
   for (int r = 0; r < 32; r += 8) Y[(long)(bx * 32 + ty + r) * ld + by * 32 + tx] = tile[tx][ty + r];
 }
-
-void launch_ydiag(hipStream_t s, const double *Dinv, double *Ydiag, int64_t ld) {
-  GOGP_KLAUNCH(ydiag_kernel<double>, dim3(64, 1, (unsigned)tl_batch.k), dim3(256), 0, s, Dinv, Ydiag,
+void launch_ydiag_zero(hipStream_t s, const double *Dinv, double *Ydiag, int64_t ld, int64_t rows_below) {
+  const unsigned nz = rows_below > 0 ? (unsigned)(rows_below / 2) : 0u;
+  GOGP_KLAUNCH(ydiag_zero_kernel<double>, dim3(64 + nz, 1, (unsigned)tl_batch.k), dim3(256), 0, s, Dinv, Ydiag,
                      (long)ld, tl_batch.stride);
 }
-void launch_ydiag(hipStream_t s, const float *Dinv, float *Ydiag, int64_t ld) {
-  GOGP_KLAUNCH(ydiag_kernel<float>, dim3(64), dim3(256), 0, s, Dinv, Ydiag, (long)ld, 0L);
+void launch_ydiag_zero(hipStream_t s, const float *Dinv, float *Ydiag, int64_t ld, int64_t rows_below) {
+  const unsigned nz = rows_below > 0 ? (unsigned)(rows_below / 2) : 0u;
+  GOGP_KLAUNCH(ydiag_zero_kernel<float>, dim3(64 + nz), dim3(256), 0, s, Dinv, Ydiag, (long)ld, 0L);
+}
+
+template <class T>
+__global__ __launch_bounds__(256) void xt_rows_kernel(const T *__restrict__ Y, long ld, T *__restrict__ X, long ldx,
+                                                      int kcols, int xtiles, long bstride) {
+  Y = cand(Y, bstride);
+  X = cand(X, bstride);
+  __shared__ T tile[32][33];
+  const int bx = blockIdx.x % xtiles, by = blockIdx.x / xtiles;
+  const int tx = threadIdx.x & 31, ty = threadIdx.x >> 5;
+  const bool zero = bx * 32 >= kcols;
+  if (!zero) {
+#pragma unroll
+    for (int r = 0; r < 32; r += 8) tile[ty + r][tx] = Y[(long)(bx * 32 + ty + r) * ld + by * 32 + tx];
+    __syncthreads();
+  }
+#pragma unroll
+  for (int r = 0; r < 32; r += 8) X[(long)(by * 32 + ty + r) * ldx + bx * 32 + tx] = zero ? (T)0 : tile[tx][ty + r];
+}
+void launch_xt_rows(hipStream_t s, const double *Y, int64_t ld, double *X, int64_t ldx, int64_t rows, int64_t kcols,
+                    int64_t xcols) {
+  if (rows <= 0 || xcols <= 0) return;
+  const int xtiles = (int)(xcols / 32);
+  GOGP_KLAUNCH(xt_rows_kernel<double>, dim3((unsigned)(xtiles * (rows / 32)), 1, (unsigned)tl_batch.k), dim3(256), 0, s, Y,
+                     (long)ld, X, (long)ldx, (int)kcols, xtiles, tl_batch.stride);
 }
 
 template <class T>
diff --git a/gogp_amd/csrc/testhooks.hip b/gogp_amd/csrc/testhooks.hip
--- a/gogp_amd/csrc/testhooks.hip
+++ b/gogp_amd/csrc/testhooks.hip
@@ -228,10 +228,11 @@
   if (K % kstep || K > (1 << 30)) return false;
   if ((mode == GEMM_LOWER || mode == GEMM_LAUUM) && mt != nt) return false;
   if (o.k < 1 || o.k > 64 || o.bstride < 0 || o.bstride % al || (o.k > 1 && o.bstride == 0)) return false;
-  if (precision == 32 && (o.k > 1 || o.kbeg0 != 0)) return false;
+  if (precision == 32 && (o.k > 1 || o.kbeg0 != 0 || o.ktri0 != 0)) return false;
   if (o.kbeg0 < 0 || o.kbeg0 % kstep || o.kbeg0 > K || (o.kbeg0 && mode != GEMM_LAUUM)) return false;
   if (o.new_row0 < -1 || (o.new_row0 >= 0 && mode != GEMM_LOWER)) return false;
   if (o.ktri && mode != GEMM_RECT) return false;
+  if (o.ktri0 < 0 || o.ktri0 > (1 << 20) || (o.ktri0 && !o.ktri)) return false;
   if (o.krag0 < -1 || (o.krag0 >= 0 && (o.ktri || (mode != GEMM_RECT && mode != GEMM_LOWER)))) return false;
   if (o.krag0 >= 0 && o.krag0 < mt && K < (int64_t)(mt - o.krag0) * TILE) return false;
   if (o.rule < 0 || o.rule > 2 || (o.rule && mode != GEMM_RECT)) return false;
@@ -240,10 +241,11 @@
     return false;
   return true;
 }
-const gogp_test_gemm_opts GEMM_OPTS_DEFAULT = {0, -1, -1, 0, 384, 0, 0, 0, 0, 0, 0, 1, 0, 1, -1, 1, 0};
+const gogp_test_gemm_opts GEMM_OPTS_DEFAULT = {0, -1, -1, 0, 384, 0, 0, 0, 0, 0, 0, 1, 0, 1, -1, 1, 0, 0};
 GemmGrid gemm_grid_of(const gogp_test_gemm_opts &o) {
   GemmGrid g;
   g.ktri = o.ktri;
+  g.ktri0 = o.ktri0;
   g.krag0 = o.krag0;
   g.new_row0 = o.new_row0;
   g.kbeg0 = o.kbeg0;
diff --git a/include/gogp_testhooks.h b/include/gogp_testhooks.h
--- a/include/gogp_testhooks.h
+++ b/include/gogp_testhooks.h
@@ -22,6 +22,7 @@
   int32_t rule, tpb_shift, rblk0, cblk0, pr, Pr, pc, Pc, beta0;
   int32_t k;
   int64_t bstride;
+  int32_t ktri0;
 } gogp_test_gemm_opts;
 
 int gogp_test_gemm_nt(int device, int precision, int mode, int mt, int nt, int64_t K, double alpha, double beta,
```

Measured after the change: 13.74 (median of 2 runs). No clear change (+0.0%).
